# ZeningLin/ViBERTgrid-PyTorch

Hardware: AMD Instinct MI355X
Metric: training docs/sec, 512x512 img + seq_len 512, bert-base+resnet34; 1/2/4/8 GPU (higher is better)
Workload: dtype f32

## Files before the change

include/vbg.h:

```cpp
#ifndef VBG_H
#define VBG_H

#ifdef __cplusplus
extern "C" {
#endif

#define VBG_VERSION 100

int vbg_version(void);

enum {
    VBG_OP_DENSE_K = 0,
    VBG_OP_DENSE_R = 1,
    VBG_OP_CONV_K = 2,
    VBG_OP_CONV_R = 3,
    VBG_OP_WT_R = 4
};
enum { VBG_EPI_NONE = 0, VBG_EPI_RELU = 1, VBG_EPI_GELU_DUAL = 2 ,
       VBG_EPI_MUL_GELU_GRAD = 3  };

typedef struct vbg_conv_geo {
    int Hs, Ws, Cs;
    int Hr, Wr;
    int kh, kw, stride, pad;
// ... 150 lines not shown
int vbg_embed_ln_bwd(const float* dout, const float* xhat, const float* rstd, const int* ids, const int* pos_ids,
                     int ntok, int hidden, const float* gamma, float drop_p, unsigned long long seed,
                     unsigned long long stream_id, float* dword, float* dpos, float* dtype0, float* dgamma,
                     float* dbeta, void* stream);
int vbg_dropout_add_ln_fwd(const float* x, const float* res, int rows, int hidden, const float* gamma,
                           const float* beta, float eps, float drop_p, unsigned long long seed,
                           unsigned long long stream_id, float* y, float* xhat, float* rstd, void* stream);
int vbg_dropout_add_ln_fwd_planes(const float* x, const float* res, int rows, int hidden, const float* gamma,
                                  const float* beta, float eps, float drop_p, unsigned long long seed,
                                  unsigned long long stream_id, float* y, float* xhat, float* rstd, unsigned short* y_planes, int ldp,
                                  long long plane, unsigned short* y_pair, int ldq, long long qplane, void* stream);
int vbg_ln_bwd_ws_rows(int rows);
int vbg_dropout_add_ln_bwd(const float* dy, const float* xhat, const float* rstd, int rows, int hidden,
                           const float* gamma, float drop_p, unsigned long long seed, unsigned long long stream_id,
                           float* dx, float* dres, float* dgamma, float* dbeta, float* slots_ws, unsigned* dx_amax, void* stream);
int vbg_dropout_add_ln_bwd_planes(const float* dy, const float* xhat, const float* rstd, int rows, int hidden,
                                  const float* gamma, float drop_p, unsigned long long seed, unsigned long long stream_id,
                                  unsigned short* dx_planes, int ldp, long long plane, float* dres, float* dgamma, float* dbeta,
                                  float* dbias_accum, float* slots3_ws, void* stream);
int vbg_dropout_add_ln_bwd_pair(const float* dy, const float* xhat, const float* rstd, int rows, int hidden,
                                const float* gamma, float drop_p, unsigned long long seed, unsigned long long stream_id,
                                unsigned short* dx_pair, int ldp, long long plane, float* dres, float* dgamma, float* dbeta,
                                float* dbias_accum, float* slots3_ws, const unsigned* dy_amax, unsigned* dx_amax, unsigned* dx_bound,
                                void* stream);
int vbg_softmax_fwd(float* s, const long long* off, const int* len, const int* ldp, int ngroups, int heads,
                    int maxlen, float scale, float drop_p, unsigned long long seed, unsigned long long stream_id,
                    void* stream);
int vbg_softmax_bwd(const float* p, float* dp, const long long* off, const int* len, const int* ldp, int ngroups,
                    int heads, int maxlen, float scale, float drop_p, void* stream);
int vbg_row_softmax(const float* x, int rows, int cols, float* y, void* stream);
int vbg_gelu_bwd(const float* h, float* dg_inout, long long n, void* stream);
int vbg_relu_bwd(const float* y, float* dy_inout, long long n, void* stream);

typedef struct vbg_planes_ref { unsigned short* buf; long long plane, ld; } vbg_planes_ref;
typedef struct vbg_bert_layer_fwd_desc {
    int ntok, hidden, inter, heads;
    float eps, drop_p; unsigned long long seed, stream_id0;
    int form_qkv, form_attn, form_ao, form_ffn;
    int tile_qkv, tile_ao, tile_ffn1, tile_ffn2;
    int ntasks, max_len; const int* tasks; const int* seq_len; const int* seq_row0; const int* pad_off; long long ntok_pad;
    const unsigned* mask_q; const unsigned* mask_k; const long long* mask_off; float attn_scale, keep_scale;
    const float* x; vbg_planes_ref xa;
    vbg_planes_ref wqkv, wo, wi, wo2;
    const float* bqkv; const float* bo; const float* bi; const float* bo2; const float* g1; const float* b1; const float* g2; const float* b2;
    vbg_planes_ref pqkv;
    float* ctx; float* lse; float* kbar; vbg_planes_ref pctx, pctxq;
    float* ao; float* x1; float* xhat1; float* rstd1; vbg_planes_ref px1, px1q;
    float* h; vbg_planes_ref pg, pgq;
    float* fo; float* y; float* xhat2; float* rstd2; vbg_planes_ref py, pyq;
} vbg_bert_layer_fwd_desc;
int vbg_bert_layer_fwd(const vbg_bert_layer_fwd_desc* desc, void* stream);

int vbg_seg_reduce_fwd(const float* tok, const int* tok_row, const int* run_start, const int* run_len, int nseg,
                       int hidden, int mode, float* out, void* stream);
int vbg_seg_reduce_bwd(const float* dout, const int* tok_row, const int* run_start, const int* run_len, int nseg,
                       int hidden, int mode, float* dtok_accum, void* stream);

int vbg_owner_map(const int* boxes, const int* box_off, int B, int gh, int gw, int stride, int* owner, void* stream);
int vbg_grid_scatter_fwd(const float* emb, const int* owner, int B, int gh, int gw, int C, int layout, float* grid,
                         void* stream);
int vbg_grid_scatter_bwd(const float* dgrid, const int* owner, const int* boxes, const int* box_doc, int nbox, int gh,
                         int gw, int stride, int C, float* demb_accum, void* stream);
int vbg_label_raster(const int* owner, const int* seg_class, long long ncell, int* pos_neg, int* cls, void* stream);

int vbg_bn_slots(void);
int vbg_bn_stats(const float* x, long long M, int C, double* slots_accum, void* stream);
int vbg_bn_finalize(double* stats, int nslots, int clear_slots, double count, const double* count_dev, int C, float eps, float momentum,
                    float* mean, float* invstd, float* running_mean, float* running_var, void* stream);
int vbg_bn_apply(const float* x, const float* res, long long M, int C, const float* mean, const float* invstd,
                 const float* gamma, const float* beta, int relu, float* y, unsigned* y_amax, void* stream);
int vbg_bn_bwd_reduce(const float* dy, const float* y, const float* x, long long M, int C, const float* mean,
                      const float* invstd, int relu, double* slots_accum, void* stream);
int vbg_bn_bwd_apply(const float* dy, const float* y, const float* x, long long M, int C, const float* mean,
                     const float* invstd, const float* gamma, const double* sums, double count, const double* count_dev,
                     int relu, float* dx,
                     float* dres, float* dgamma_accum, float* dbeta_accum, unsigned* dx_amax, void* stream);
int vbg_bn_apply_fold(const float* x, const float* res, long long M, int C, double* slots, int nslots, double count,
                      const double* count_dev, float eps, float momentum, float* mean, float* invstd, float* running_mean,
                      float* running_var, const float* gamma, const float* beta, int relu, float* y, unsigned* y_amax, void* stream);
int vbg_bn_fold_count(double* slots, int nslots, int clear_slots, int C, double* folded, double count, void* stream);
int vbg_bn_bwd_apply_fold(const float* dy, const float* y, const float* x, long long M, int C, const float* mean,
                          const float* invstd, const float* gamma, double* slots, int nslots, double count, int relu, float* dx,
                          float* dres, float* dgamma_accum, float* dbeta_accum, unsigned* dx_amax, void* stream);
int vbg_bn_param_grad(double* slots, int nslots, int clear_slots, int C, double* folded, float* dgamma_accum, float* dbeta_accum,
                      void* stream);
int vbg_maxpool3x3s2_fwd(const float* x, int B, int H, int W, int C, float* y, int* argmax, void* stream);
int vbg_maxpool3x3s2_bwd(const float* dy, const int* argmax, int B, int Ho, int Wo, int C, int H, int W,
                         float* dx, void* stream);
int vbg_avgpool2_fwd(const float* x, int B, int H, int W, int C, float* y, void* stream);
int vbg_avgpool2_bwd(const float* dy, int B, int H, int W, int C, float* dx, void* stream);
int vbg_upsample2_add(const float* lo, const float* skip, int B, int H, int W, int C, float* y, void* stream);
int vbg_sumpool(const float* hi, int B, int H, int W, int C, int f, float* lo, int accumulate, void* stream);
int vbg_nchw_to_nhwc(const float* x, int B, int C, int HW, float* y, void* stream);
int vbg_nhwc_to_nchw(const float* x, int B, int C, int HW, float* y, void* stream);
int vbg_upsample_nhwc_to_nchw(const float* x, int B, int h, int w, int C, int f, float* y, void* stream);
int vbg_add_inplace(float* a, const float* b, long long n, void* stream);

int vbg_roi_align_fwd(const float* feat, int B, int H, int W, int C, const int* boxes, const int* box_doc, int nroi,
                      int out, float scale, float* y , void* stream);
int vbg_roi_align_bwd(const float* dy, int B, int H, int W, int C, const int* boxes, const int* box_doc, int nroi,
                      int out, float scale, float* dfeat_accum, void* stream);
int vbg_roi_align_hw_fwd(const float* feat, int B, int H, int W, int C, const int* boxes, const int* box_doc, int nroi,
                         int out_h, int out_w, float scale, float* y, void* stream);
int vbg_roi_align_hw_bwd(const float* dy, int B, int H, int W, int C, const int* boxes, const int* box_doc, int nroi,
                         int out_h, int out_w, float scale, float* dfeat_accum, void* stream);

int vbg_ce_fwd(const float* logits, long long ld, int ncls, const int* elem, const int* labels, long long n,
               const float* weight, int up_shift, int H, int W, float* loss, void* stream);
int vbg_ce_bwd(const float* logits, long long ld, int ncls, const int* elem, const int* labels, long long n,
               const float* weight, const float* gscale_dev, float gmul, int up_shift, int H, int W,
               float* dlogits_accum, void* stream);
long long vbg_compact_ws_bytes(long long n);
int vbg_compact(const int* labels, long long n, int value, int eq, int* out_idx, int* out_count_dev, void* ws,
                long long ws_bytes, void* stream);
long long vbg_sort_ws_bytes(long long n);
int vbg_sort_desc(const float* keys, long long n, float* keys_out, int* idx_out, void* ws, long long ws_bytes,
                  void* stream);
int vbg_gather_f32(const float* src, const int* idx, long long n, float* out, void* stream);
int vbg_gather_i32(const int* src, const int* idx, long long n, int* out, void* stream);
int vbg_sum_f32(const float* x, long long n, float* out_accum, void* stream);

int vbg_gather_rows(const float* src, const int* idx, long long n, int C, float* dst, void* stream);
int vbg_scatter_rows_add(const float* src, const int* idx, long long n, int C, float* dst_accum, void* stream);
int vbg_crf_nll_fwd(const float* emissions, const int* tags, const int* doc_off, int ndoc, const float* trans, int ntag,
                    int start_tag, int stop_tag, float* alpha, float* logz, float* nll, void* stream);
int vbg_crf_nll_bwd(const float* emissions, const int* tags, const int* doc_off, int ndoc, const float* trans, int ntag,
                    int start_tag, int stop_tag, const float* alpha, const float* logz, const float* gout, float* demissions,
                    float* dtrans_accum, void* stream);
int vbg_crf_viterbi(const float* emissions, const int* doc_off, int ndoc, const float* trans, int ntag, int start_tag,
                    int stop_tag, int* backptr, int* path, float* score, void* stream);

int vbg_sgd_step(float* p, const float* g, float* mom, long long n, float lr, float momentum, float wd,
                 int first_step, float grad_scale, void* stream);
int vbg_adamw_step(float* p, const float* g, float* m, float* v, long long n, float lr, float b1, float b2,
                   float eps, float wd, int step, float grad_scale, void* stream);
int vbg_sumsq(const float* g, long long n, float* out_accum, void* stream);
int vbg_scale_inplace(float* x, long long n, float s, void* stream);

long long vbg_colsum_det_ws_elems(long long M, int N);
int vbg_colsum_det(const float* x, long long ld, long long M, int N, float* out, int accumulate, double* ws, void* stream);
int vbg_sum_det_ws_elems(void);
int vbg_sum_det(const float* x, long long n, int squares, float* out_accum, float* ws, void* stream);
long long vbg_sort_i32_ws_bytes(long long n);
int vbg_sort_i32(const int* keys, long long n, int* keys_out, int* idx_out, void* ws, long long ws_bytes, void* stream);
int vbg_segment_rows_add(const float* src, long long lds, const int* perm, const int* sorted_keys, long long n, int C,
                         float* dst_accum, long long ldd, void* stream);
int vbg_ce_bwd_rows(const float* logits, long long ld, int ncls, const int* elem, const int* labels, long long n,
                    const float* weight, const float* gscale_dev, float gmul, int up_shift, int H, int W, float* grow, int* keys,
                    void* stream);
int vbg_roi_align_bwd_det(const float* dy, int B, int H, int W, int C, const int* boxes, const int* box_doc, int nroi, int out,
                          float scale, float* dfeat_accum, void* stream);
int vbg_roi_align_hw_bwd_det(const float* dy, int B, int H, int W, int C, const int* boxes, const int* box_doc, int nroi, int out_h,
                             int out_w, float scale, float* dfeat_accum, void* stream);
int vbg_bn_det_ws_rows(long long M, int C);
int vbg_bn_stats_det(const float* x, long long M, int C, double* ws, double* zero_slots, void* stream);
int vbg_bn_bwd_reduce_det(const float* dy, const float* y, const float* x, long long M, int C, const float* mean,
                          const float* invstd, int relu, double* ws, double* zero_slots, void* stream);
int vbg_embed_ln_bwd_det_blocks(int ntok);
int vbg_embed_ln_bwd_det(const float* dout, const float* xhat, const float* rstd, int ntok, int hidden, const float* gamma,
                         float drop_p, unsigned long long seed, unsigned long long sid, float* dz_rows, float* part, void* stream);
int vbg_crf_nll_bwd_det(const float* emissions, const int* tags, const int* doc_off, int ndoc, const float* trans, int ntag,
                        int start_tag, int stop_tag, const float* alpha, const float* logz, const float* gout, float* demissions,
                        float* dtrans_part, void* stream);

#ifdef __cplusplus
}
#endif
#endif
```

vibertgrid-pytorch_amd/csrc/convaux.hip:

```cpp
#include "vbg_common.h"
#include "../../include/vbg.h"

namespace vbg {

static inline int ew_grid(long long n, int block) {
    long long g = (n + block - 1) / block;
    if (g > 256 * 8) g = 256 * 8;
    if (g < 1) g = 1;
    return (int)g;
}

constexpr int BN_SLOTS = 32;
template <bool BWD, bool STORE = false>
__global__ __launch_bounds__(256) void bn_reduce_kernel(const float* __restrict__ a, const float* __restrict__ y,
                                                        const float* __restrict__ x, long long M, int C,
                                                        const float* __restrict__ mean, const float* __restrict__ invstd,
                                                        int relu, int rows_per_block, double* out) {
    __shared__ double sh[2][256][4];
    const int C4 = C >> 2;
    const int QB = min(C4, 64);
    const int RL = 256 / QB;
    const int q = threadIdx.x % QB, rl = threadIdx.x / QB;
    const int cq = blockIdx.x * 64 + q;
    const long long r0 = (long long)blockIdx.y * rows_per_block;
    const long long r1 = min(M, r0 + rows_per_block);
    float4 s = make_float4(0.f, 0.f, 0.f, 0.f), t = make_float4(0.f, 0.f, 0.f, 0.f);
    if (cq < C4 && rl < RL) {
        float4 mu = make_float4(0.f, 0.f, 0.f, 0.f), is = mu;
        if (BWD) { mu = reinterpret_cast<const float4*>(mean)[cq]; is = reinterpret_cast<const float4*>(invstd)[cq]; }
#pragma unroll 4
        for (long long r = r0 + rl; r < r1; r += RL) {
            const long long o = r * C4 + cq;
            float4 v = reinterpret_cast<const float4*>(a)[o];
            if (!BWD) {
                s.x += v.x; s.y += v.y; s.z += v.z; s.w += v.w;
                t.x += v.x * v.x; t.y += v.y * v.y; t.z += v.z * v.z; t.w += v.w * v.w;
            } else {
                if (relu) {
                    const float4 yv = reinterpret_cast<const float4*>(y)[o];
                    v.x = yv.x > 0.f ? v.x : 0.f; v.y = yv.y > 0.f ? v.y : 0.f;
                    v.z = yv.z > 0.f ? v.z : 0.f; v.w = yv.w > 0.f ? v.w : 0.f;
                }
                const float4 xv = reinterpret_cast<const float4*>(x)[o];
                s.x += v.x; s.y += v.y; s.z += v.z; s.w += v.w;
                t.x += v.x * ((xv.x - mu.x) * is.x); t.y += v.y * ((xv.y - mu.y) * is.y);
                t.z += v.z * ((xv.z - mu.z) * is.z); t.w += v.w * ((xv.w - mu.w) * is.w);
            }
        }
    }
    sh[0][threadIdx.x][0] = s.x; sh[0][threadIdx.x][1] = s.y; sh[0][threadIdx.x][2] = s.z; sh[0][threadIdx.x][3] = s.w;
    sh[1][threadIdx.x][0] = t.x; sh[1][threadIdx.x][1] = t.y; sh[1][threadIdx.x][2] = t.z; sh[1][threadIdx.x][3] = t.w;
    __syncthreads();
    if (rl == 0 && cq < C4) {
        double a0[4] = {0, 0, 0, 0}, a1[4] = {0, 0, 0, 0};
        for (int l = 0; l < RL; ++l)
#pragma unroll
            for (int j = 0; j < 4; ++j) { a0[j] += sh[0][l * QB + q][j]; a1[j] += sh[1][l * QB + q][j]; }
        double* o = out + (size_t)(STORE ? blockIdx.y : blockIdx.y % BN_SLOTS) * 2 * C;
#pragma unroll
        for (int j = 0; j < 4; ++j) {
            if (STORE) {
                o[cq * 4 + j] = a0[j];
                o[C + cq * 4 + j] = a1[j];
            } else {
                unsafeAtomicAdd(o + cq * 4 + j, a0[j]);
                unsafeAtomicAdd(o + C + cq * 4 + j, a1[j]);
            }
        }
    }
}

static inline int bn_rows_per_block(long long M, int C) {
    const int C4 = C / 4, QB = C4 < 64 ? C4 : 64, RL = 256 / QB, CG = cdiv(C4, 64);
    long long r = cdiv(M * CG, 512);
    if (r < 2 * RL) r = 2 * RL;
    r = cdiv(r, RL) * RL;
    return (int)r;
}

__device__ __forceinline__ double fold_slots(double* __restrict__ slots, int nslots, int C, int idx, bool clear) {
    double v[4] = {0.0, 0.0, 0.0, 0.0};
    int s = 0;
#pragma unroll 2
    for (; s + 3 < nslots; s += 4) {
#pragma unroll
        for (int j = 0; j < 4; ++j) v[j] += slots[(size_t)(s + j) * 2 * C + idx];
    }
    for (; s < nslots; ++s) v[0] += slots[(size_t)s * 2 * C + idx];
    if (clear)
        for (s = 0; s < nslots; ++s) slots[(size_t)s * 2 * C + idx] = 0.0;
    return (v[0] + v[1]) + (v[2] + v[3]);
}

__global__ void bn_finalize_kernel(double* __restrict__ stats, int nslots, int clear, double count, const double* __restrict__ count_dev, int C,
                                   float eps, float momentum, float* mean, float* invstd, float* running_mean,
                                   float* running_var) {
    const int c = blockIdx.x * blockDim.x + threadIdx.x;
    if (c >= C) return;
    if (count_dev) count = count_dev[0];
    const double m = fold_slots(stats, nslots, C, c, clear) / count;
    double var = fold_slots(stats, nslots, C, C + c, clear) / count - m * m;
    if (var < 0.0) var = 0.0;
    mean[c] = (float)m;
    invstd[c] = (float)(1.0 / sqrt(var + (double)eps));
    if (running_mean) {
        const double unbiased = count > 1.0 ? var * count / (count - 1.0) : var;
        running_mean[c] = (1.f - momentum) * running_mean[c] + momentum * (float)m;
        running_var[c] = (1.f - momentum) * running_var[c] + momentum * (float)unbiased;
    }
}

__device__ __forceinline__ void amax_publish(float mx, unsigned* amax) {
    __shared__ float amax_sh[16];
#pragma unroll
    for (int o = 32; o > 0; o >>= 1) mx = fmaxf(mx, __shfl_xor(mx, o, 64));
    if ((threadIdx.x & 63) == 0) amax_sh[threadIdx.x >> 6] = mx;
    __syncthreads();
    if (threadIdx.x == 0) {
        for (int w = 1; w < (int)(blockDim.x >> 6); ++w) mx = fmaxf(mx, amax_sh[w]);
        const unsigned bits = __float_as_uint(mx);
        unsigned* word = amax + (blockIdx.x & (VBG_AMAX_WORDS - 1)) * VBG_AMAX_STRIDE;
        if (bits > __hip_atomic_load(word, __ATOMIC_RELAXED, __HIP_MEMORY_SCOPE_AGENT)) atomicMax(word, bits);
    }
}

__global__ void bn_apply_kernel(const float* __restrict__ x, const float* __restrict__ res, long long M, int C4,
                                const float* __restrict__ mean, const float* __restrict__ invstd,
                                const float* __restrict__ gamma, const float* __restrict__ beta, int relu,
                                float* __restrict__ y, unsigned* amax) {
    const long long total = M * C4;
    const long long stride = (long long)gridDim.x * blockDim.x;
    float mx = 0.f;
    for (long long i = (long long)blockIdx.x * blockDim.x + threadIdx.x; i < total; i += stride) {
        const int c4 = (int)(i % C4);
        const float4 xv = reinterpret_cast<const float4*>(x)[i];
        const float4 mu = reinterpret_cast<const float4*>(mean)[c4];
        const float4 is = reinterpret_cast<const float4*>(invstd)[c4];
        const float4 ga = reinterpret_cast<const float4*>(gamma)[c4];
        const float4 be = reinterpret_cast<const float4*>(beta)[c4];
        float4 o;
        o.x = (xv.x - mu.x) * is.x * ga.x + be.x; o.y = (xv.y - mu.y) * is.y * ga.y + be.y;
        o.z = (xv.z - mu.z) * is.z * ga.z + be.z; o.w = (xv.w - mu.w) * is.w * ga.w + be.w;
        if (res) {
            const float4 rv = reinterpret_cast<const float4*>(res)[i];
            o.x += rv.x; o.y += rv.y; o.z += rv.z; o.w += rv.w;
        }
        if (relu) { o.x = fmaxf(o.x, 0.f); o.y = fmaxf(o.y, 0.f); o.z = fmaxf(o.z, 0.f); o.w = fmaxf(o.w, 0.f); }
        reinterpret_cast<float4*>(y)[i] = o;
        mx = fmaxf(fmaxf(mx, fmaxf(fabsf(o.x), fabsf(o.y))), fmaxf(fabsf(o.z), fabsf(o.w)));
    }
    if (amax) amax_publish(mx, amax);
}

__global__ void bn_bwd_apply_kernel(const float* __restrict__ dy, const float* __restrict__ y, const float* __restrict__ x,
                                    long long M, int C4, int C, const float* __restrict__ mean, const float* __restrict__ invstd,
                                    const float* __restrict__ gamma, const double* __restrict__ sums, double count,
                                    const double* __restrict__ count_dev, int relu, float* __restrict__ dx,
                                    float* __restrict__ dres, unsigned* amax) {
    if (count_dev) count = count_dev[0];
    float mx = 0.f;
    const float icnt = (float)(1.0 / count);
    const long long total = M * C4;
    const long long stride = (long long)gridDim.x * blockDim.x;
    for (long long i = (long long)blockIdx.x * blockDim.x + threadIdx.x; i < total; i += stride) {
        const int c4 = (int)(i % C4), c = c4 * 4;
        float4 g = reinterpret_cast<const float4*>(dy)[i];
        if (relu) {
            const float4 yv = reinterpret_cast<const float4*>(y)[i];
            g.x = yv.x > 0.f ? g.x : 0.f; g.y = yv.y > 0.f ? g.y : 0.f; g.z = yv.z > 0.f ? g.z : 0.f; g.w = yv.w > 0.f ? g.w : 0.f;
        }
        const float4 xv = reinterpret_cast<const float4*>(x)[i];
        const float4 mu = reinterpret_cast<const float4*>(mean)[c4], is = reinterpret_cast<const float4*>(invstd)[c4];
        const float4 ga = reinterpret_cast<const float4*>(gamma)[c4];
        float4 o;
        o.x = ga.x * is.x * (g.x - (float)sums[c + 0] * icnt - (xv.x - mu.x) * is.x * ((float)sums[C + c + 0] * icnt));
        o.y = ga.y * is.y * (g.y - (float)sums[c + 1] * icnt - (xv.y - mu.y) * is.y * ((float)sums[C + c + 1] * icnt));
        o.z = ga.z * is.z * (g.z - (float)sums[c + 2] * icnt - (xv.z - mu.z) * is.z * ((float)sums[C + c + 2] * icnt));
        o.w = ga.w * is.w * (g.w - (float)sums[c + 3] * icnt - (xv.w - mu.w) * is.w * ((float)sums[C + c + 3] * icnt));
        reinterpret_cast<float4*>(dx)[i] = o;
        if (dres) reinterpret_cast<float4*>(dres)[i] = g;
        mx = fmaxf(fmaxf(mx, fmaxf(fabsf(o.x), fabsf(o.y))), fmaxf(fabsf(o.z), fabsf(o.w)));
    }
    if (amax) amax_publish(mx, amax);
}

__device__ __forceinline__ void amax_publish_at(float mx, unsigned* amax, unsigned block_id) {
    __shared__ float amax_sh2[16];
#pragma unroll
    for (int o = 32; o > 0; o >>= 1) mx = fmaxf(mx, __shfl_xor(mx, o, 64));
    if ((threadIdx.x & 63) == 0) amax_sh2[threadIdx.x >> 6] = mx;
    __syncthreads();
    if (threadIdx.x == 0) {
        for (int w = 1; w < (int)(blockDim.x >> 6); ++w) mx = fmaxf(mx, amax_sh2[w]);
        const unsigned bits = __float_as_uint(mx);
        unsigned* word = amax + (block_id & (VBG_AMAX_WORDS - 1)) * VBG_AMAX_STRIDE;
        if (bits > __hip_atomic_load(word, __ATOMIC_RELAXED, __HIP_MEMORY_SCOPE_AGENT)) atomicMax(word, bits);
    }
}

__global__ __launch_bounds__(256) void bn_apply_fold_kernel(const float* __restrict__ x, const float* __restrict__ res, long long M, int C,
                                                            double* __restrict__ slots, int nslots, double count,
                                                            const double* __restrict__ count_dev, float eps, float momentum,
                                                            float* __restrict__ mean_out, float* __restrict__ invstd_out,
                                                            float* __restrict__ running_mean, float* __restrict__ running_var,
                                                            const float* __restrict__ gamma, const float* __restrict__ beta, int relu,
                                                            int rows_per_block, float* __restrict__ y, unsigned* amax) {
    __shared__ double fold[128];
    __shared__ __attribute__((aligned(16))) float cst[4][64];
    const int tid = threadIdx.x, c0 = blockIdx.y * 64;
    if (count_dev) count = count_dev[0];
    if (tid < 128) fold[tid] = fold_slots(slots, nslots, C, (tid >> 6) * C + c0 + (tid & 63), false);
    __syncthreads();
    if (tid < 64) {
        const int c = c0 + tid;
        const double m = fold[tid] / count;
        double var = fold[64 + tid] / count - m * m;
        if (var < 0.0) var = 0.0;
        const float mf = (float)m, isf = (float)(1.0 / sqrt(var + (double)eps));
        cst[0][tid] = mf; cst[1][tid] = isf; cst[2][tid] = gamma[c]; cst[3][tid] = beta[c];
        if (blockIdx.x == 0) {
            mean_out[c] = mf;
            invstd_out[c] = isf;
            if (running_mean) {
                const double unbiased = count > 1.0 ? var * count / (count - 1.0) : var;
                running_mean[c] = (1.f - momentum) * running_mean[c] + momentum * mf;
                running_var[c] = (1.f - momentum) * running_var[c] + momentum * (float)unbiased;
            }
        }
    }
    __syncthreads();
    const int q = tid & 15, rl = tid >> 4, C4 = C >> 2, cq = blockIdx.y * 16 + q;
    const float4 mu = reinterpret_cast<const float4*>(cst[0])[q], is = reinterpret_cast<const float4*>(cst[1])[q];
    const float4 ga = reinterpret_cast<const float4*>(cst[2])[q], be = reinterpret_cast<const float4*>(cst[3])[q];
    const long long r0 = (long long)blockIdx.x * rows_per_block, r1 = min(M, r0 + rows_per_block);
    float mx = 0.f;
#pragma unroll 4
    for (long long r = r0 + rl; r < r1; r += 16) {
        const long long i = r * C4 + cq;
        const float4 xv = reinterpret_cast<const float4*>(x)[i];
        float4 o;
        o.x = (xv.x - mu.x) * is.x * ga.x + be.x; o.y = (xv.y - mu.y) * is.y * ga.y + be.y;
        o.z = (xv.z - mu.z) * is.z * ga.z + be.z; o.w = (xv.w - mu.w) * is.w * ga.w + be.w;
        if (res) {
            const float4 rv = reinterpret_cast<const float4*>(res)[i];
            o.x += rv.x; o.y += rv.y; o.z += rv.z; o.w += rv.w;
        }
        if (relu) { o.x = fmaxf(o.x, 0.f); o.y = fmaxf(o.y, 0.f); o.z = fmaxf(o.z, 0.f); o.w = fmaxf(o.w, 0.f); }
        reinterpret_cast<float4*>(y)[i] = o;
        mx = fmaxf(fmaxf(mx, fmaxf(fabsf(o.x), fabsf(o.y))), fmaxf(fabsf(o.z), fabsf(o.w)));
    }
    if (amax) amax_publish_at(mx, amax, blockIdx.x + blockIdx.y * gridDim.x);
}

__global__ __launch_bounds__(256) void bn_bwd_apply_fold_kernel(const float* __restrict__ dy, const float* __restrict__ y,
                                                                const float* __restrict__ x, long long M, int C,
                                                                const float* __restrict__ mean, const float* __restrict__ invstd,
                                                                const float* __restrict__ gamma, double* __restrict__ slots, int nslots,
                                                                double count, int relu, int rows_per_block, float* __restrict__ dx,
                                                                float* __restrict__ dres, float* dgamma, float* dbeta, unsigned* amax) {
    __shared__ double fold[128];
    __shared__ __attribute__((aligned(16))) float cst[5][64];
    const int tid = threadIdx.x, c0 = blockIdx.y * 64;
    if (tid < 128) fold[tid] = fold_slots(slots, nslots, C, (tid >> 6) * C + c0 + (tid & 63), false);
    __syncthreads();
    const float icnt = (float)(1.0 / count);
    if (tid < 64) {
        const int c = c0 + tid;
        const double sg = fold[tid], sgx = fold[64 + tid];
        cst[0][tid] = mean[c]; cst[1][tid] = invstd[c]; cst[2][tid] = gamma[c];
        cst[3][tid] = (float)sg * icnt; cst[4][tid] = (float)sgx * icnt;
        if (blockIdx.x == 0) {
            if (dbeta) dbeta[c] += (float)sg;
            if (dgamma) dgamma[c] += (float)sgx;
        }
    }
    __syncthreads();
    const int q = tid & 15, rl = tid >> 4, C4 = C >> 2, cq = blockIdx.y * 16 + q;
    const float4 mu = reinterpret_cast<const float4*>(cst[0])[q], is = reinterpret_cast<const float4*>(cst[1])[q];
    const float4 ga = reinterpret_cast<const float4*>(cst[2])[q], s0 = reinterpret_cast<const float4*>(cst[3])[q];
    const float4 s1 = reinterpret_cast<const float4*>(cst[4])[q];
    const long long r0 = (long long)blockIdx.x * rows_per_block, r1 = min(M, r0 + rows_per_block);
    float mx = 0.f;
#pragma unroll 4
    for (long long r = r0 + rl; r < r1; r += 16) {
        const long long i = r * C4 + cq;
        float4 g = reinterpret_cast<const float4*>(dy)[i];
        if (relu) {
            const float4 yv = reinterpret_cast<const float4*>(y)[i];
            g.x = yv.x > 0.f ? g.x : 0.f; g.y = yv.y > 0.f ? g.y : 0.f; g.z = yv.z > 0.f ? g.z : 0.f; g.w = yv.w > 0.f ? g.w : 0.f;
        }
        const float4 xv = reinterpret_cast<const float4*>(x)[i];
        float4 o;
        o.x = ga.x * is.x * (g.x - s0.x - (xv.x - mu.x) * is.x * s1.x);
        o.y = ga.y * is.y * (g.y - s0.y - (xv.y - mu.y) * is.y * s1.y);
        o.z = ga.z * is.z * (g.z - s0.z - (xv.z - mu.z) * is.z * s1.z);
        o.w = ga.w * is.w * (g.w - s0.w - (xv.w - mu.w) * is.w * s1.w);
        reinterpret_cast<float4*>(dx)[i] = o;
        if (dres) reinterpret_cast<float4*>(dres)[i] = g;
        mx = fmaxf(fmaxf(mx, fmaxf(fabsf(o.x), fabsf(o.y))), fmaxf(fabsf(o.z), fabsf(o.w)));
    }
    if (amax) amax_publish_at(mx, amax, blockIdx.x + blockIdx.y * gridDim.x);
}

__global__ __launch_bounds__(256) void amax_kernel(const float* __restrict__ x, long long n, unsigned* amax) {
    const long long n4 = n / 4, stride = (long long)gridDim.x * blockDim.x;
    float mx = 0.f;
    for (long long i = (long long)blockIdx.x * blockDim.x + threadIdx.x; i < n4; i += stride) {
        const float4 v = reinterpret_cast<const float4*>(x)[i];
        mx = fmaxf(fmaxf(mx, fmaxf(fabsf(v.x), fabsf(v.y))), fmaxf(fabsf(v.z), fabsf(v.w)));
    }
    if (blockIdx.x == 0 && threadIdx.x < (int)(n - n4 * 4)) mx = fmaxf(mx, fabsf(x[n4 * 4 + threadIdx.x]));
    amax_publish(mx, amax);
}

__global__ void bn_param_grad_kernel(double* __restrict__ slots, int nslots, int clear, int C, double* __restrict__ folded, float* dgamma,
                                     float* dbeta, double tail = -1.0) {
    const int c = blockIdx.x * blockDim.x + threadIdx.x;
    if (c == 0 && folded && tail >= 0.0) folded[2 * C] = tail;
    if (c >= C) return;
    const double sg = fold_slots(slots, nslots, C, c, clear), sgx = fold_slots(slots, nslots, C, C + c, clear);
    if (folded) { folded[c] = sg; folded[C + c] = sgx; }
    if (dbeta) dbeta[c] += (float)sg;
    if (dgamma) dgamma[c] += (float)sgx;
}

__global__ void maxpool_fwd_kernel(const float* __restrict__ x, int B, int H, int W, int C, int Ho, int Wo,
                                   float* __restrict__ y, int* __restrict__ argmax) {
    const long long total = (long long)B * Ho * Wo * C;
    const long long stride = (long long)gridDim.x * blockDim.x;
    for (long long i = (long long)blockIdx.x * blockDim.x + threadIdx.x; i < total; i += stride) {
        const int c = (int)(i % C);
        long long t = i / C;
        const int ox = (int)(t % Wo); t /= Wo;
        const int oy = (int)(t % Ho);
        const int b = (int)(t / Ho);
        float best = -INFINITY;
        int bi = -1;
        for (int dy = 0; dy < 3; ++dy) {
            const int iy = oy * 2 - 1 + dy;
            if (iy < 0 || iy >= H) continue;
            for (int dx = 0; dx < 3; ++dx) {
                const int ix = ox * 2 - 1 + dx;
                if (ix < 0 || ix >= W) continue;
                const float v = x[(((long long)b * H + iy) * W + ix) * C + c];
                if (v > best || bi < 0) { best = v; bi = iy * W + ix; }
            }
        }
        y[i] = best;
        argmax[i] = bi;
    }
}

__global__ void maxpool_bwd_kernel(const float* __restrict__ dy, const int* __restrict__ argmax, int B, int Ho, int Wo, int C4, int H,
                                   int W, float* __restrict__ dx) {
    const long long total = (long long)B * H * W * C4;
    const long long stride = (long long)gridDim.x * blockDim.x;
    for (long long i = (long long)blockIdx.x * blockDim.x + threadIdx.x; i < total; i += stride) {
        const int c4 = (int)(i % C4);
        long long t = i / C4;
        const int x = (int)(t % W); t /= W;
        const int y = (int)(t % H);
        const int b = (int)(t / H);
        const int me = y * W + x;
        float4 g = make_float4(0.f, 0.f, 0.f, 0.f);
        for (int oy = y >> 1; oy <= ((y + 1) >> 1); ++oy) {
            if (oy >= Ho) continue;
            for (int ox = x >> 1; ox <= ((x + 1) >> 1); ++ox) {
                if (ox >= Wo) continue;
                const long long o = (((long long)b * Ho + oy) * Wo + ox) * C4 + c4;
                const int4 am = reinterpret_cast<const int4*>(argmax)[o];
                const float4 d = reinterpret_cast<const float4*>(dy)[o];
                g.x += am.x == me ? d.x : 0.f; g.y += am.y == me ? d.y : 0.f;
// ... 102 lines not shown
    const long long total = (long long)B * C * H * W;
    const long long stride = (long long)gridDim.x * blockDim.x;
    for (long long i = (long long)blockIdx.x * blockDim.x + threadIdx.x; i < total; i += stride) {
        const int X = (int)(i % W);
        long long t = i / W;
        const int Y = (int)(t % H); t /= H;
        const int c = (int)(t % C);
        const int b = (int)(t / C);
        y[i] = x[(((long long)b * h + Y / f) * w + X / f) * C + c];
    }
}

__global__ void normalize_resize_kernel(const float* __restrict__ img, int h, int w, int oh, int ow, float m0, float m1, float m2,
                                        float s0, float s1, float s2, float* __restrict__ out, int W) {
    const int i = blockIdx.x * blockDim.x + threadIdx.x;
    if (i >= oh * ow) return;
    const int oy = i / ow, ox = i - oy * ow;
    const float mean[3] = {m0, m1, m2}, sd[3] = {s0, s1, s2};
    float v[3];
    if (oh == h && ow == w) {
#pragma unroll
        for (int c = 0; c < 3; ++c) v[c] = (img[((long long)c * h + oy) * w + ox] - mean[c]) / sd[c];
    } else {
        const float sy = (float)h / (float)oh, sx = (float)w / (float)ow;
        float fy = ((float)oy + 0.5f) * sy - 0.5f; if (fy < 0.f) fy = 0.f;
        float fx = ((float)ox + 0.5f) * sx - 0.5f; if (fx < 0.f) fx = 0.f;
        const int y0 = (int)fy, x0 = (int)fx;
        const int y1 = y0 + ((y0 < h - 1) ? 1 : 0), x1 = x0 + ((x0 < w - 1) ? 1 : 0);
        const float ly = fy - (float)y0, lx = fx - (float)x0, hy = 1.f - ly, hx = 1.f - lx;
#pragma unroll
        for (int c = 0; c < 3; ++c) {
            const float* p = img + (long long)c * h * w;
            const float a = (p[(long long)y0 * w + x0] - mean[c]) / sd[c], b = (p[(long long)y0 * w + x1] - mean[c]) / sd[c];
            const float d = (p[(long long)y1 * w + x0] - mean[c]) / sd[c], e = (p[(long long)y1 * w + x1] - mean[c]) / sd[c];
            v[c] = hy * (hx * a + lx * b) + ly * (hx * d + lx * e);
        }
    }
    float* o = out + ((long long)oy * W + ox) * 3;
    o[0] = v[0]; o[1] = v[1]; o[2] = v[2];
}

__global__ void rescale_boxes_kernel(const long long* __restrict__ in, int n, float rh, float rw, int* __restrict__ out) {
    const int i = blockIdx.x * blockDim.x + threadIdx.x;
    if (i >= n) return;
    const float r = ((i & 1) == 0) ? rh : rw;
    out[i] = (int)__fmul_rn((float)in[i], r);
}

__global__ void im2col_kernel(const float* __restrict__ x, int B, int H, int W, int C, int kh, int kw, int stride, int pad,
                              int Ho, int Wo, int Kpad, float* __restrict__ out) {
    const int KQ = Kpad >> 2, K = kh * kw * C;
    const long long total = (long long)B * Ho * Wo * KQ;
    const long long gstride = (long long)gridDim.x * blockDim.x;
    for (long long i = (long long)blockIdx.x * blockDim.x + threadIdx.x; i < total; i += gstride) {
        const long long pix = i / KQ;
        const int k0 = (int)(i - pix * KQ) * 4;
        const int p = (int)pix;
        const int ox = p % Wo, t = p / Wo, oy = t % Ho, b = t / Ho;
        const float* img = x + (long long)b * H * W * C;
        float v[4];
#pragma unroll
        for (int j = 0; j < 4; ++j) {
            const int k = k0 + j;
            v[j] = 0.f;
            if (k < K) {
                const int tap = k / C, c = k - tap * C;
                const int dy = tap / kw, dx = tap - dy * kw;
                const int iy = oy * stride - pad + dy, ix = ox * stride - pad + dx;
                if (iy >= 0 && iy < H && ix >= 0 && ix < W) v[j] = img[(iy * W + ix) * C + c];
            }
        }
        reinterpret_cast<float4*>(out)[i] = make_float4(v[0], v[1], v[2], v[3]);
    }
}

}

using namespace vbg;
#define S_ ((hipStream_t)stream)
#define ALIGNED16(p) (((uintptr_t)(p)) % 16 == 0)

extern "C" int vbg_bn_stats(const float* x, long long M, int C, double* stats_accum, void* stream) {
    VBG_CHECK_ARG(x && stats_accum && M >= 0 && C > 0 && C % 4 == 0 && ALIGNED16(x));
    VBG_CHECK_ARG(C / 4 <= 64 ? (256 % (C / 4) == 0) : (C / 4) % 64 == 0);
    if (M == 0) return VBG_OK;
    const int rpb = bn_rows_per_block(M, C);
    VBG_LAUNCH((bn_reduce_kernel<false>), dim3(cdiv(C / 4, 64), cdiv(M, rpb)), dim3(256), 0, S_, x, nullptr, nullptr, M, C, nullptr,
               nullptr, 0, rpb, stats_accum);
    VBG_LAUNCH_RET();
}

extern "C" int vbg_bn_slots(void) { return BN_SLOTS; }

extern "C" int vbg_bn_finalize(double* stats, int nslots, int clear_slots, double count, const double* count_dev, int C, float eps, float momentum,
                               float* mean, float* invstd, float* running_mean, float* running_var, void* stream) {
    VBG_CHECK_ARG(stats && nslots >= 1 && mean && invstd && C > 0 && (count > 0 || count_dev) &&
                  ((running_mean == nullptr) == (running_var == nullptr)));
    VBG_LAUNCH(bn_finalize_kernel, dim3(cdiv(C, 256)), dim3(256), 0, S_, stats, nslots, clear_slots, count, count_dev, C, eps, momentum, mean,
                       invstd, running_mean, running_var);
    VBG_LAUNCH_RET();
}

extern "C" int vbg_bn_apply(const float* x, const float* res, long long M, int C, const float* mean, const float* invstd,
                            const float* gamma, const float* beta, int relu, float* y, unsigned* y_amax, void* stream) {
    VBG_CHECK_ARG(x && mean && invstd && gamma && beta && y && M >= 0 && C > 0 && C % 4 == 0);
    VBG_CHECK_ARG(ALIGNED16(x) && ALIGNED16(y) && ALIGNED16(mean) && ALIGNED16(invstd) && ALIGNED16(gamma) && ALIGNED16(beta) &&
                  (!res || ALIGNED16(res)));
    if (M == 0) return VBG_OK;
    VBG_LAUNCH(bn_apply_kernel, dim3(ew_grid(M * (C / 4), 256)), dim3(256), 0, S_, x, res, M, C / 4, mean, invstd, gamma,
                       beta, relu, y, y_amax);
    VBG_LAUNCH_RET();
}

extern "C" int vbg_bn_bwd_reduce(const float* dy, const float* y, const float* x, long long M, int C, const float* mean,
                                 const float* invstd, int relu, double* sums_accum, void* stream) {
    VBG_CHECK_ARG(dy && x && mean && invstd && sums_accum && M >= 0 && C > 0 && (!relu || y) && C % 4 == 0);
    VBG_CHECK_ARG(ALIGNED16(dy) && ALIGNED16(x) && ALIGNED16(mean) && ALIGNED16(invstd) && (!relu || ALIGNED16(y)));
    VBG_CHECK_ARG(C / 4 <= 64 ? (256 % (C / 4) == 0) : (C / 4) % 64 == 0);
    if (M == 0) return VBG_OK;
    const int rpb = bn_rows_per_block(M, C);
    VBG_LAUNCH((bn_reduce_kernel<true>), dim3(cdiv(C / 4, 64), cdiv(M, rpb)), dim3(256), 0, S_, dy, y, x, M, C, mean, invstd, relu,
               rpb, sums_accum);
    VBG_LAUNCH_RET();
}

extern "C" int vbg_bn_bwd_apply(const float* dy, const float* y, const float* x, long long M, int C, const float* mean,
                                const float* invstd, const float* gamma, const double* sums, double count,
                                const double* count_dev, int relu, float* dx, float* dres, float* dgamma_accum,
                                float* dbeta_accum, unsigned* dx_amax, void* stream) {
    VBG_CHECK_ARG(dy && x && mean && invstd && gamma && sums && dx && M >= 0 && C > 0 && (count > 0 || count_dev) && (!relu || y));
    VBG_CHECK_ARG(C % 4 == 0 && ALIGNED16(dy) && ALIGNED16(x) && ALIGNED16(dx) && ALIGNED16(mean) && ALIGNED16(invstd) &&
                  ALIGNED16(gamma) && (!relu || ALIGNED16(y)) && (!dres || ALIGNED16(dres)));
    if (M > 0) VBG_LAUNCH(bn_bwd_apply_kernel, dim3(ew_grid(M * (C / 4), 256)), dim3(256), 0, S_, dy, y, x, M, C / 4, C, mean, invstd,
                          gamma, sums, count, count_dev, relu, dx, dres, dx_amax);
    if (dgamma_accum && dbeta_accum)
        VBG_LAUNCH(bn_param_grad_kernel, dim3(cdiv(C, 256)), dim3(256), 0, S_, const_cast<double*>(sums), 1, 0, C, (double*)nullptr, dgamma_accum, dbeta_accum, -1.0);
    VBG_LAUNCH_RET();
}

static inline int bn_fold_rows(long long M, int C) {
    long long r = cdiv(M * (C / 64), 1536);
    if (r < 64) r = 64;
    return (int)(cdiv(r, 16) * 16);
}

extern "C" int vbg_bn_apply_fold(const float* x, const float* res, long long M, int C, double* slots, int nslots, double count,
                                 const double* count_dev, float eps, float momentum, float* mean, float* invstd, float* running_mean,
                                 float* running_var, const float* gamma, const float* beta, int relu, float* y, unsigned* y_amax, void* stream) {
    VBG_CHECK_ARG(x && y && slots && mean && invstd && gamma && beta && M > 0 && C > 0 && C % 64 == 0 && nslots >= 1 && (count > 0 || count_dev));
    VBG_CHECK_ARG((running_mean == nullptr) == (running_var == nullptr) && ALIGNED16(x) && ALIGNED16(y) && (!res || ALIGNED16(res)));
    const int rpb = bn_fold_rows(M, C);
    VBG_LAUNCH(bn_apply_fold_kernel, dim3(cdiv(M, rpb), C / 64), dim3(256), 0, S_, x, res, M, C, slots, nslots, count, count_dev, eps, momentum, mean, invstd,
               running_mean, running_var, gamma, beta, relu, rpb, y, y_amax);
    VBG_LAUNCH_RET();
}

extern "C" int vbg_bn_bwd_apply_fold(const float* dy, const float* y, const float* x, long long M, int C, const float* mean,
                                     const float* invstd, const float* gamma, double* slots, int nslots, double count, int relu, float* dx,
                                     float* dres, float* dgamma_accum, float* dbeta_accum, unsigned* dx_amax, void* stream) {
    VBG_CHECK_ARG(dy && x && mean && invstd && gamma && slots && dx && M > 0 && C > 0 && C % 64 == 0 && nslots >= 1 && count > 0 && (!relu || y));
    VBG_CHECK_ARG(((dgamma_accum == nullptr) == (dbeta_accum == nullptr)) && ALIGNED16(dy) && ALIGNED16(x) && ALIGNED16(dx) &&
                  (!relu || ALIGNED16(y)) && (!dres || ALIGNED16(dres)));
    const int rpb = bn_fold_rows(M, C);
    VBG_LAUNCH(bn_bwd_apply_fold_kernel, dim3(cdiv(M, rpb), C / 64), dim3(256), 0, S_, dy, y, x, M, C, mean, invstd, gamma, slots, nslots, count,
               relu, rpb, dx, dres, dgamma_accum, dbeta_accum, dx_amax);
    VBG_LAUNCH_RET();
}

extern "C" int vbg_amax(const float* x, long long n, unsigned* amax, void* stream) {
    VBG_CHECK_ARG(n >= 0 && amax);
    if (n == 0) return VBG_OK;
    VBG_CHECK_ARG(x && ALIGNED16(x));
    VBG_LAUNCH(amax_kernel, dim3(ew_grid((n + 3) / 4, 256 * 8)), dim3(256), 0, S_, x, n, amax);
    VBG_LAUNCH_RET();
}

extern "C" int vbg_bn_param_grad(double* slots, int nslots, int clear_slots, int C, double* folded, float* dgamma_accum,
                                 float* dbeta_accum, void* stream) {
    VBG_CHECK_ARG(slots && nslots >= 1 && C > 0 && ((dgamma_accum == nullptr) == (dbeta_accum == nullptr)) && (folded || dgamma_accum));
    VBG_LAUNCH(bn_param_grad_kernel, dim3(cdiv(C, 256)), dim3(256), 0, S_, slots, nslots, clear_slots, C, folded, dgamma_accum, dbeta_accum, -1.0);
    VBG_LAUNCH_RET();
}

extern "C" int vbg_bn_fold_count(double* slots, int nslots, int clear_slots, int C, double* folded, double count, void* stream) {
    VBG_CHECK_ARG(slots && folded && nslots >= 1 && C > 0 && count >= 0);
    VBG_LAUNCH(bn_param_grad_kernel, dim3(cdiv(C, 256)), dim3(256), 0, S_, slots, nslots, clear_slots, C, folded, (float*)nullptr, (float*)nullptr, count);
    VBG_LAUNCH_RET();
}

extern "C" int vbg_maxpool3x3s2_fwd(const float* x, int B, int H, int W, int C, float* y, int* argmax, void* stream) {
    VBG_CHECK_ARG(x && y && argmax && B >= 0 && H > 0 && W > 0 && C > 0);
    const int Ho = (H + 2 - 3) / 2 + 1, Wo = (W + 2 - 3) / 2 + 1;
    const long long total = (long long)B * Ho * Wo * C;
    if (total == 0) return VBG_OK;
    VBG_LAUNCH(maxpool_fwd_kernel, dim3(ew_grid(total, 256)), dim3(256), 0, S_, x, B, H, W, C, Ho, Wo, y, argmax);
    VBG_LAUNCH_RET();
}

extern "C" int vbg_maxpool3x3s2_bwd(const float* dy, const int* argmax, int B, int Ho, int Wo, int C, int H, int W,
                                    float* dx_zeroed, void* stream) {
    VBG_CHECK_ARG(dy && argmax && dx_zeroed && B >= 0 && Ho > 0 && Wo > 0 && C > 0 && C % 4 == 0);
    VBG_CHECK_ARG(ALIGNED16(dy) && ALIGNED16(argmax) && ALIGNED16(dx_zeroed) && Ho == (H + 2 - 3) / 2 + 1 && Wo == (W + 2 - 3) / 2 + 1);
    const long long total = (long long)B * Ho * Wo * C;
    if (total == 0) return VBG_OK;
    VBG_LAUNCH(maxpool_bwd_kernel, dim3(ew_grid((long long)B * H * W * (C / 4), 256)), dim3(256), 0, S_, dy, argmax, B, Ho, Wo, C / 4, H, W,
               dx_zeroed);
    VBG_LAUNCH_RET();
}

extern "C" int vbg_upsample2_add(const float* lo, const float* skip, int B, int H, int W, int C, float* y, void* stream) {
    VBG_CHECK_ARG(lo && skip && y && H % 2 == 0 && W % 2 == 0 && C % 4 == 0 && ALIGNED16(lo) && ALIGNED16(skip) && ALIGNED16(y));
    const long long total = (long long)B * H * W * (C / 4);
    if (total == 0) return VBG_OK;
    VBG_LAUNCH(upsample2_add_kernel, dim3(ew_grid(total, 256)), dim3(256), 0, S_, lo, skip, B, H, W, C / 4, y);
    VBG_LAUNCH_RET();
}

extern "C" int vbg_avgpool2_fwd(const float* x, int B, int H, int W, int C, float* y, void* stream) {
    VBG_CHECK_ARG(x && y && B >= 0 && H >= 2 && W >= 2 && C > 0 && C % 4 == 0 && ALIGNED16(x) && ALIGNED16(y));
    const long long total = (long long)B * (H / 2) * (W / 2) * (C / 4);
    if (total == 0) return VBG_OK;
    VBG_LAUNCH((avgpool2_kernel<false>), dim3(ew_grid(total, 256)), dim3(256), 0, S_, x, B, H, W, C / 4, y);
    VBG_LAUNCH_RET();
}

extern "C" int vbg_avgpool2_bwd(const float* dy, int B, int H, int W, int C, float* dx, void* stream) {
    VBG_CHECK_ARG(dy && dx && B >= 0 && H >= 2 && W >= 2 && C > 0 && C % 4 == 0 && ALIGNED16(dy) && ALIGNED16(dx));
    const long long total = (long long)B * H * W * (C / 4);
    if (total == 0) return VBG_OK;
    VBG_LAUNCH((avgpool2_kernel<true>), dim3(ew_grid(total, 256)), dim3(256), 0, S_, dy, B, H, W, C / 4, dx);
    VBG_LAUNCH_RET();
}

extern "C" int vbg_sumpool(const float* hi, int B, int H, int W, int C, int f, float* lo, int accumulate, void* stream) {
    VBG_CHECK_ARG(hi && lo && f >= 1 && H % f == 0 && W % f == 0 && C % 4 == 0 && ALIGNED16(hi) && ALIGNED16(lo));
    const long long total = (long long)B * (H / f) * (W / f) * (C / 4);
    if (total == 0) return VBG_OK;
    VBG_LAUNCH(sumpool_kernel, dim3(ew_grid(total, 256)), dim3(256), 0, S_, hi, B, H, W, C / 4, f, lo, accumulate);
    VBG_LAUNCH_RET();
}

extern "C" int vbg_nchw_to_nhwc(const float* x, int B, int C, int HW, float* y, void* stream) {
    VBG_CHECK_ARG(x && y && B >= 0 && C > 0 && HW > 0);
    if (B == 0) return VBG_OK;
    VBG_LAUNCH(transpose_kernel, dim3(cdiv(HW, 32), cdiv(C, 32), B), dim3(256), 0, S_, x, C, HW, y);
    VBG_LAUNCH_RET();
}

extern "C" int vbg_nhwc_to_nchw(const float* x, int B, int C, int HW, float* y, void* stream) {
    VBG_CHECK_ARG(x && y && B >= 0 && C > 0 && HW > 0);
    if (B == 0) return VBG_OK;
    VBG_LAUNCH(transpose_kernel, dim3(cdiv(C, 32), cdiv(HW, 32), B), dim3(256), 0, S_, x, HW, C, y);
    VBG_LAUNCH_RET();
}

extern "C" int vbg_upsample_nhwc_to_nchw(const float* x, int B, int h, int w, int C, int f, float* y, void* stream) {
    VBG_CHECK_ARG(x && y && f >= 1 && C > 0);
    const long long total = (long long)B * C * h * f * w * f;
    if (total == 0) return VBG_OK;
    VBG_LAUNCH(upsample_nhwc_to_nchw_kernel, dim3(ew_grid(total, 256)), dim3(256), 0, S_, x, B, h, w, C, f, y);
    VBG_LAUNCH_RET();
}

extern "C" int vbg_normalize_resize(const float* img, int h, int w, int oh, int ow, const float* h_mean3, const float* h_std3,
                                    float* batch_nhwc, int b, int H, int W, void* stream) {
    VBG_CHECK_ARG(img && h_mean3 && h_std3 && batch_nhwc && h > 0 && w > 0 && oh > 0 && ow > 0 && oh <= H && ow <= W && b >= 0);
    float* out = batch_nhwc + (long long)b * H * W * 3;
    VBG_LAUNCH(normalize_resize_kernel, dim3(cdiv((long)oh * ow, 256)), dim3(256), 0, S_, img, h, w, oh, ow, h_mean3[0],
                       h_mean3[1], h_mean3[2], h_std3[0], h_std3[1], h_std3[2], out, W);
    VBG_LAUNCH_RET();
}

extern "C" int vbg_rescale_boxes(const long long* in, int S, float ratio_h, float ratio_w, int* out, void* stream) {
    VBG_CHECK_ARG(S >= 0);
    if (S == 0) return VBG_OK;
    VBG_CHECK_ARG(in && out);
    VBG_LAUNCH(rescale_boxes_kernel, dim3(cdiv(S * 4, 256)), dim3(256), 0, S_, in, S * 4, ratio_h, ratio_w, out);
    VBG_LAUNCH_RET();
}

extern "C" int vbg_im2col(const float* x, int B, int H, int W, int C, int kh, int kw, int stride, int pad, int Kpad, float* out,
                          void* stream) {
    VBG_CHECK_ARG(x && out && Kpad >= kh * kw * C && Kpad % 4 == 0 && stride > 0 && ALIGNED16(out));
    const int Ho = (H + 2 * pad - kh) / stride + 1, Wo = (W + 2 * pad - kw) / stride + 1;
    VBG_CHECK_ARG((long long)B * Ho * Wo < (1ll << 31) && (long long)H * W * C < (1ll << 31));
    const long long total = (long long)B * Ho * Wo * (Kpad / 4);
    if (total == 0) return VBG_OK;
    VBG_LAUNCH(im2col_kernel, dim3(ew_grid(total, 256)), dim3(256), 0, S_, x, B, H, W, C, kh, kw, stride, pad, Ho, Wo, Kpad,
                       out);
    VBG_LAUNCH_RET();
}

__global__ void bn_det_fold_kernel(const double* __restrict__ ws, int nblk, int C2, double* __restrict__ slot0) {
    const int i = blockIdx.x * blockDim.x + threadIdx.x;
    if (i >= C2) return;
    double s = 0.0;
    for (int k = 0; k < nblk; ++k) s += ws[(long long)k * C2 + i];
    slot0[i] = s;
}

extern "C" int vbg_bn_det_ws_rows(long long M, int C) {
    if (M <= 0 || C <= 0 || C % 4 != 0) return 0;
    return cdiv(M, bn_rows_per_block(M, C));
}

extern "C" int vbg_bn_stats_det(const float* x, long long M, int C, double* ws, double* zero_slots, void* stream) {
    VBG_CHECK_ARG(x && ws && zero_slots && M >= 0 && C > 0 && C % 4 == 0 && ALIGNED16(x));
    VBG_CHECK_ARG(C / 4 <= 64 ? (256 % (C / 4) == 0) : (C / 4) % 64 == 0);
    if (M == 0) return VBG_OK;
    const int rpb = bn_rows_per_block(M, C), nblk = cdiv(M, rpb);
    VBG_LAUNCH((bn_reduce_kernel<false, true>), dim3(cdiv(C / 4, 64), nblk), dim3(256), 0, S_, x, nullptr, nullptr, M, C, nullptr,
               nullptr, 0, rpb, ws);
    VBG_LAUNCH(bn_det_fold_kernel, dim3(cdiv(2 * C, 256)), dim3(256), 0, S_, ws, nblk, 2 * C, zero_slots);
    VBG_LAUNCH_RET();
}

extern "C" int vbg_bn_bwd_reduce_det(const float* dy, const float* y, const float* x, long long M, int C, const float* mean,
                                     const float* invstd, int relu, double* ws, double* zero_slots, void* stream) {
    VBG_CHECK_ARG(dy && x && mean && invstd && ws && zero_slots && M >= 0 && C > 0 && (!relu || y) && C % 4 == 0);
    VBG_CHECK_ARG(ALIGNED16(dy) && ALIGNED16(x) && ALIGNED16(mean) && ALIGNED16(invstd) && (!relu || ALIGNED16(y)));
    VBG_CHECK_ARG(C / 4 <= 64 ? (256 % (C / 4) == 0) : (C / 4) % 64 == 0);
    if (M == 0) return VBG_OK;
    const int rpb = bn_rows_per_block(M, C), nblk = cdiv(M, rpb);
    VBG_LAUNCH((bn_reduce_kernel<true, true>), dim3(cdiv(C / 4, 64), nblk), dim3(256), 0, S_, dy, y, x, M, C, mean, invstd, relu,
               rpb, ws);
    VBG_LAUNCH(bn_det_fold_kernel, dim3(cdiv(2 * C, 256)), dim3(256), 0, S_, ws, nblk, 2 * C, zero_slots);
    VBG_LAUNCH_RET();
}
```

vibertgrid-pytorch_amd/csrc/gemm_planes.hip:

```cpp
#include "vbg_common.h"
#include <type_traits>
#include <cstdlib>
#include <hip/hip_ext.h>
#include "../../include/vbg.h"

namespace vbg {

typedef unsigned pg_u32x4 __attribute__((ext_vector_type(4)));
typedef __bf16 pg_bf16x8 __attribute__((ext_vector_type(8)));
constexpr unsigned PG_INVALID = 0x80000000u;

__device__ __forceinline__ __amdgpu_buffer_rsrc_t pg_rsrc(const void* base) {
    return __builtin_amdgcn_make_buffer_rsrc(const_cast<void*>(base), 0, (int)0x80000000u, 0x00020000);
}

typedef _Float16 pg_f16x8 __attribute__((ext_vector_type(8)));
__device__ __forceinline__ void pg_split2(float a, float b, unsigned& hi, unsigned& lo) {
    typedef float f32x2_t __attribute__((ext_vector_type(2)));
    typedef _Float16 f16x2_t __attribute__((ext_vector_type(2)));
    const f32x2_t v = {a, b};
    const f16x2_t h = __builtin_convertvector(v, f16x2_t);
    const f16x2_t l = __builtin_convertvector((v - __builtin_convertvector(h, f32x2_t)) * 2048.f, f16x2_t);
    hi = __builtin_bit_cast(unsigned, h);
    lo = __builtin_bit_cast(unsigned, l);
// ... 608 lines not shown
                const float4 hv = *reinterpret_cast<const float4*>(C2 + (long long)gm * ldc + gn);
                v.x *= gelu_erf_grad(hv.x); v.y *= gelu_erf_grad(hv.y); v.z *= gelu_erf_grad(hv.z); v.w *= gelu_erf_grad(hv.w);
            }
            if (C) *reinterpret_cast<float4*>(cp) = v;
            if (epi == VBG_EPI_GELU_DUAL) {
                v = make_float4(gelu_erf(v.x), gelu_erf(v.y), gelu_erf(v.z), gelu_erf(v.w));
                if (C2) *reinterpret_cast<float4*>(C2 + (long long)gm * ldc + gn) = v;
            }
            if (Cp) {
                const float e[4] = {v.x, v.y, v.z, v.w};
                unsigned short h[4], m[4], l[4];
#pragma unroll
                for (int t = 0; t < 4; ++t) pg_split3(e[t], h[t], m[t], l[t]);
                unsigned short* o = Cp + (long long)gm * p.ldp + gn;
                *reinterpret_cast<uint2*>(o) = make_uint2(h[0] | ((unsigned)h[1] << 16), h[2] | ((unsigned)h[3] << 16));
                *reinterpret_cast<uint2*>(o + p.c_plane) = make_uint2(m[0] | ((unsigned)m[1] << 16), m[2] | ((unsigned)m[3] << 16));
                *reinterpret_cast<uint2*>(o + 2 * p.c_plane) = make_uint2(l[0] | ((unsigned)l[1] << 16), l[2] | ((unsigned)l[3] << 16));
            }
        }
        __syncthreads();
    }
}

__device__ __forceinline__ void pg_split3(float x, unsigned short& h, unsigned short& m, unsigned short& l) {
    const unsigned u = __float_as_uint(x);
    const float r1 = x - __uint_as_float(u & 0xffff0000u);
    const unsigned u1 = __float_as_uint(r1);
    const float r2 = r1 - __uint_as_float(u1 & 0xffff0000u);
    h = (unsigned short)(u >> 16); m = (unsigned short)(u1 >> 16); l = (unsigned short)(__float_as_uint(r2) >> 16);
}

__global__ __launch_bounds__(256) void split_planes_kernel(const float* __restrict__ x, long long ldx, int rows, int cols,
                                                            unsigned short* __restrict__ out, int ldp, long long plane, int relu,
                                                            float* colsum) {
    extern __shared__ float sh_cols[];
    const int cpr = ldp / 8;
    const long long n = (long long)rows * cpr;
    const long long stride = (long long)gridDim.x * blockDim.x;
    float cs[8] = {0.f, 0.f, 0.f, 0.f, 0.f, 0.f, 0.f, 0.f};
    const long long i0 = (long long)blockIdx.x * blockDim.x + threadIdx.x;
    for (long long i = i0; i < n; i += stride) {
        const int r = (int)(i / cpr), c = (int)(i % cpr) * 8;
        float e[8];
        if (c + 8 <= cols && ((ldx & 3) == 0) && ((((uintptr_t)x) & 15) == 0)) {
            const float4 a = *reinterpret_cast<const float4*>(x + (long long)r * ldx + c);
            const float4 b = *reinterpret_cast<const float4*>(x + (long long)r * ldx + c + 4);
            e[0] = a.x; e[1] = a.y; e[2] = a.z; e[3] = a.w; e[4] = b.x; e[5] = b.y; e[6] = b.z; e[7] = b.w;
        } else {
#pragma unroll
            for (int t = 0; t < 8; ++t) e[t] = (c + t < cols) ? x[(long long)r * ldx + c + t] : 0.f;
        }
        unsigned short h[8], m[8], l[8];
#pragma unroll
        for (int t = 0; t < 8; ++t) {
            cs[t] += e[t];
            pg_split3(relu ? fmaxf(e[t], 0.f) : e[t], h[t], m[t], l[t]);
        }
        unsigned short* o = out + (long long)r * ldp + c;
        auto pack = [](const unsigned short* s) {
            return make_uint4(s[0] | ((unsigned)s[1] << 16), s[2] | ((unsigned)s[3] << 16), s[4] | ((unsigned)s[5] << 16), s[6] | ((unsigned)s[7] << 16));
        };
        *reinterpret_cast<uint4*>(o) = pack(h);
        *reinterpret_cast<uint4*>(o + plane) = pack(m);
        *reinterpret_cast<uint4*>(o + 2 * plane) = pack(l);
    }
    if (colsum) {
        for (int c = threadIdx.x; c < ldp; c += blockDim.x) sh_cols[c] = 0.f;
        __syncthreads();
        if (i0 < n) {
            const int c = (int)(i0 % cpr) * 8;
#pragma unroll
            for (int t = 0; t < 8; ++t) atomicAdd(&sh_cols[c + t], cs[t]);
        }
        __syncthreads();
        for (int c = threadIdx.x; c < cols; c += blockDim.x) {
            const float v = sh_cols[c];
            if (v != 0.f) unsafeAtomicAdd(colsum + c, v);
        }
    }
}

__global__ __launch_bounds__(256) void split_planes_pair_kernel(const float* __restrict__ x, long long ldx, int rows, int cols,
                                                                 unsigned short* __restrict__ out, int ldp, long long plane,
                                                                 const unsigned* amax, float* colsum) {
    extern __shared__ float sh_cols[];
    const float sc = amax ? vbg_pow2_scale(vbg_amax_read(amax)).x : 1.f;
    float cs[8] = {0.f, 0.f, 0.f, 0.f, 0.f, 0.f, 0.f, 0.f};
    const long long i0 = (long long)blockIdx.x * blockDim.x + threadIdx.x;
    const int cpr = ldp / 8;
    const long long n = (long long)rows * cpr;
    const long long stride = (long long)gridDim.x * blockDim.x;
    const bool vec = ((ldx & 3) == 0) && ((((uintptr_t)x) & 15) == 0);
    for (long long i = (long long)blockIdx.x * blockDim.x + threadIdx.x; i < n; i += stride) {
        const int r = (int)(i / cpr), c = (int)(i % cpr) * 8;
        float e[8];
        if (c + 8 <= cols && vec) {
            const float4 a = *reinterpret_cast<const float4*>(x + (long long)r * ldx + c);
            const float4 b = *reinterpret_cast<const float4*>(x + (long long)r * ldx + c + 4);
            e[0] = a.x; e[1] = a.y; e[2] = a.z; e[3] = a.w; e[4] = b.x; e[5] = b.y; e[6] = b.z; e[7] = b.w;
        } else {
#pragma unroll
            for (int t = 0; t < 8; ++t) e[t] = (c + t < cols) ? x[(long long)r * ldx + c + t] : 0.f;
        }
#pragma unroll
        for (int t = 0; t < 8; ++t) { cs[t] += e[t]; e[t] *= sc; }
        uint4 h, l;
        pg_split2(e[0], e[1], h.x, l.x); pg_split2(e[2], e[3], h.y, l.y); pg_split2(e[4], e[5], h.z, l.z); pg_split2(e[6], e[7], h.w, l.w);
        unsigned short* o = out + (long long)r * ldp + c;
        *reinterpret_cast<uint4*>(o) = h;
        *reinterpret_cast<uint4*>(o + plane) = l;
    }
    if (colsum) {
        for (int c = threadIdx.x; c < ldp; c += blockDim.x) sh_cols[c] = 0.f;
        __syncthreads();
        if (i0 < n) {
            const int c = (int)(i0 % cpr) * 8;
#pragma unroll
            for (int t = 0; t < 8; ++t) atomicAdd(&sh_cols[c + t], cs[t]);
        }
        __syncthreads();
        for (int c = threadIdx.x; c < cols; c += blockDim.x) {
            const float v = sh_cols[c];
            if (v != 0.f) unsafeAtomicAdd(colsum + c, v);
        }
    }
}

__global__ __launch_bounds__(256) void col_l1_max_kernel(const vbg_l1_entry* __restrict__ tab, unsigned* __restrict__ out) {
    const vbg_l1_entry e = tab[blockIdx.y];
    const int c0 = blockIdx.x * 64;
    if (c0 >= e.cols) return;
    const int tx = threadIdx.x & 15, ty = threadIdx.x >> 4;
    const int c = c0 + tx * 4;
    const bool vec = (e.ld & 3) == 0 && ((((uintptr_t)e.w) & 15) == 0) && c + 4 <= e.cols;
    float4 s = make_float4(0.f, 0.f, 0.f, 0.f);
#pragma unroll 4
    for (int r = ty; r < e.rows; r += 16) {
        const float* p = e.w + (long long)r * e.ld + c;
        if (vec) {
            const float4 v = *reinterpret_cast<const float4*>(p);
            s.x += fabsf(v.x); s.y += fabsf(v.y); s.z += fabsf(v.z); s.w += fabsf(v.w);
        } else {
            if (c < e.cols) s.x += fabsf(p[0]);
            if (c + 1 < e.cols) s.y += fabsf(p[1]);
            if (c + 2 < e.cols) s.z += fabsf(p[2]);
            if (c + 3 < e.cols) s.w += fabsf(p[3]);
        }
    }
    __shared__ float4 red[16][16];
    red[ty][tx] = s;
    __syncthreads();
    if (ty == 0) {
        float4 t = red[0][tx];
#pragma unroll
        for (int g = 1; g < 16; ++g) { const float4 v = red[g][tx]; t.x += v.x; t.y += v.y; t.z += v.z; t.w += v.w; }
        float m = fmaxf(fmaxf(t.x, t.y), fmaxf(t.z, t.w));
#pragma unroll
        for (int o = 8; o > 0; o >>= 1) m = fmaxf(m, __shfl_xor(m, o, 64));
        if (tx == 0) atomicMax(out + blockIdx.y, __float_as_uint(m));
    }
}

__global__ __launch_bounds__(256) void split_planes_t_kernel(const float* __restrict__ x, long long ldx, int rows, int cols,
                                                              unsigned short* __restrict__ out, int ldp, long long plane) {
    __shared__ float t[64][65];
    const int r0 = blockIdx.x * 64, c0 = blockIdx.y * 64;
    const int tid = threadIdx.x;
    const bool vec = ((ldx & 3) == 0) && ((((uintptr_t)x) & 15) == 0);
#pragma unroll
    for (int i = 0; i < 4; ++i) {
        const int f = tid + i * 256, r = f / 16, c = (f % 16) * 4;
        float4 v = make_float4(0.f, 0.f, 0.f, 0.f);
        if (r0 + r < rows) {
            const float* src = x + (long long)(r0 + r) * ldx + c0 + c;
            if (vec && c0 + c + 4 <= cols) v = *reinterpret_cast<const float4*>(src);
            else {
                if (c0 + c + 0 < cols) v.x = src[0];
                if (c0 + c + 1 < cols) v.y = src[1];
                if (c0 + c + 2 < cols) v.z = src[2];
                if (c0 + c + 3 < cols) v.w = src[3];
            }
        }
        t[r][c] = v.x; t[r][c + 1] = v.y; t[r][c + 2] = v.z; t[r][c + 3] = v.w;
    }
    __syncthreads();
#pragma unroll
    for (int i = 0; i < 2; ++i) {
        const int f = tid + i * 256, c = f / 8, rg = (f % 8) * 8;
        if (c0 + c >= cols || r0 + rg >= ldp) continue;
        unsigned short h[8], m[8], l[8];
#pragma unroll
        for (int e = 0; e < 8; ++e) pg_split3(t[rg + e][c], h[e], m[e], l[e]);
        unsigned short* o = out + (long long)(c0 + c) * ldp + r0 + rg;
        auto pack = [](const unsigned short* s) {
            return make_uint4(s[0] | ((unsigned)s[1] << 16), s[2] | ((unsigned)s[3] << 16), s[4] | ((unsigned)s[5] << 16), s[6] | ((unsigned)s[7] << 16));
        };
        *reinterpret_cast<uint4*>(o) = pack(h);
        *reinterpret_cast<uint4*>(o + plane) = pack(m);
        *reinterpret_cast<uint4*>(o + 2 * plane) = pack(l);
    }
}

template <bool PAIR>
__global__ __launch_bounds__(256) void split_planes_t_batched_kernel(const float* __restrict__ src, unsigned short* __restrict__ dst,
                                                                      const long long* __restrict__ tbl, int njobs, long long plane) {
    __shared__ float t[64][65];
    int j = 0;
// ... 135 lines not shown
            if (tile == 256128) pg_launch_pair<256, 128, 4, 2, 3, true>(d, s, ev0, ev1);
            else pg_launch_pair<128, 128, 4, 2, 3, true>(d, s, ev0, ev1);
            VBG_LAUNCH_RET();
        }
        if (tile == 256128) pg_launch_pair<256, 128, 4, 2, 3>(d, s, ev0, ev1);
        else if (tile == 128130) pg_launch_pair<128, 128, 2, 4, 3>(d, s, ev0, ev1);
        else if (tile == 128129 || tile == 0) pg_launch_pair<128, 128, 4, 2, 4>(d, s, ev0, ev1);
        else if ((tile == 64064 || tile == 64004) && d.ngroups == 0 && !d.c_amax && !d.cq_ref_in && !d.colsum) {
            if (tile == 64004) pg_launch_pair<64, 64, 2, 2, 4>(d, s, ev0, ev1);
            else pg_launch_pair<64, 64, 2, 2, 3>(d, s, ev0, ev1);
        } else return VBG_EARG;
        VBG_LAUNCH_RET();
    }
    VBG_CHECK_ARG(d.form == 0);
    if (d.trans) {
        if (tile == 256128) pg_launch<256, 128, 4, 2, 2, true>(d, s, (hipEvent_t)e0, (hipEvent_t)e1);
        else if (tile == 128130) pg_launch<128, 128, 2, 4, 3, true>(d, s, (hipEvent_t)e0, (hipEvent_t)e1);
        else pg_launch<128, 128, 4, 2, 3, true>(d, s, (hipEvent_t)e0, (hipEvent_t)e1);
        VBG_LAUNCH_RET();
    }
    if (tile == 0) {
        const long t128 = (long)cdiv(d.M, 128) * cdiv(d.N, 128) * d.splitk;
        tile = (t128 >= 200 && d.N >= 128) ? 128128 : 64064;
    }
    if (tile == 256256) {
        VBG_CHECK_ARG(d.splitk == 1 && !d.accumulate && d.K % 16 == 0);
        const dim3 g(cdiv(d.M, 256), cdiv(d.N, 256));
        (void)hipGetLastError();
        hipEvent_t ev0 = (hipEvent_t)e0, ev1 = (hipEvent_t)e1;
        if (ev0 && ev1) hipExtLaunchKernelGGL(plane_gemm_256_kernel, g, dim3(512), 0, s, ev0, ev1, 0, d);
        else hipLaunchKernelGGL(plane_gemm_256_kernel, g, dim3(512), 0, s, d);
        VBG_LAUNCH_RET();
    }
    if (tile == 256128) pg_launch<256, 128, 4, 2, 2>(d, s, (hipEvent_t)e0, (hipEvent_t)e1);
    else if (tile == 128128) pg_launch<128, 128, 2, 2, 3>(d, s, (hipEvent_t)e0, (hipEvent_t)e1);
    else if (tile == 128129) pg_launch<128, 128, 4, 2, 3>(d, s, (hipEvent_t)e0, (hipEvent_t)e1);
    else if (tile == 128130) pg_launch<128, 128, 2, 4, 3>(d, s, (hipEvent_t)e0, (hipEvent_t)e1);
    else if (tile == 128064) pg_launch<128, 64, 2, 2, 3>(d, s, (hipEvent_t)e0, (hipEvent_t)e1);
    else if (tile == 64064) pg_launch<64, 64, 2, 2, 3>(d, s, (hipEvent_t)e0, (hipEvent_t)e1);
    else return VBG_EARG;
    VBG_LAUNCH_RET();
}

extern "C" int vbg_plane_gemm(const vbg_plane_gemm_desc* desc, void* stream) { return plane_gemm_dispatch(desc, stream, nullptr, nullptr); }

extern "C" int vbg_plane_gemm_timed(const vbg_plane_gemm_desc* desc, void* stream, void* start_event, void* stop_event) {
    VBG_CHECK_ARG(start_event && stop_event);
    return plane_gemm_dispatch(desc, stream, start_event, stop_event);
}

extern "C" int vbg_split_planes(const float* x, long long ldx, int rows, int cols, unsigned short* out, int ldp, long long plane,
                                int relu, float* colsum_accum, void* stream) {
    VBG_CHECK_ARG(rows >= 0 && cols >= 0 && ldp % 32 == 0 && ldp >= cols && plane >= (long long)rows * ldp && plane % 8 == 0);
    if (rows == 0 || cols == 0) return VBG_OK;
    VBG_CHECK_ARG(x && out && ((uintptr_t)out & 15) == 0);
    const long long n = (long long)rows * (ldp / 8);
    long long g = (n + 255) / 256;
    size_t lds = 0;
    if (colsum_accum) {
        VBG_CHECK_ARG(relu == 0 && ldp * 4 <= 64 * 1024);
        const long long cpr = ldp / 8;
        long long a = cpr, b = 256;
        while (b) { const long long t = a % b; a = b; b = t; }
        const long long unit = cpr / a;
        long long k = 288 / unit;
        if (k < 1) k = 1;
        const long long need = (g + unit - 1) / unit;
        if (k > need) k = need;
        g = k * unit;
        lds = (size_t)ldp * 4;
    } else if (g > 256 * 16) {
        g = 256 * 16;
    }
    VBG_LAUNCH(split_planes_kernel, dim3((unsigned)g), dim3(256), lds, (hipStream_t)stream, x, ldx, rows, cols, out, ldp, plane, relu,
               colsum_accum);
    VBG_LAUNCH_RET();
}

extern "C" int vbg_split_planes_pair(const float* x, long long ldx, int rows, int cols, unsigned short* out, int ldp, long long plane,
                                     const unsigned* amax, float* colsum_accum, void* stream) {
    VBG_CHECK_ARG(rows >= 0 && cols >= 0 && ldp % 32 == 0 && ldp >= cols && plane >= (long long)rows * ldp && plane % 8 == 0);
    if (rows == 0 || cols == 0) return VBG_OK;
    VBG_CHECK_ARG(x && out && ((uintptr_t)out & 15) == 0);
    const long long n = (long long)rows * (ldp / 8);
    long long g = (n + 255) / 256;
    size_t lds = 0;
    if (colsum_accum) {
        VBG_CHECK_ARG(ldp * 4 <= 64 * 1024);
        const long long cpr = ldp / 8;
        long long a = cpr, b = 256;
        while (b) { const long long t = a % b; a = b; b = t; }
        const long long unit = cpr / a;
        long long k = 288 / unit;
        if (k < 1) k = 1;
        const long long need = (g + unit - 1) / unit;
        if (k > need) k = need;
        g = k * unit;
        lds = (size_t)ldp * 4;
    } else if (g > 256 * 16) {
        g = 256 * 16;
    }
    VBG_LAUNCH(split_planes_pair_kernel, dim3((unsigned)g), dim3(256), lds, (hipStream_t)stream, x, ldx, rows, cols, out, ldp, plane, amax, colsum_accum);
    VBG_LAUNCH_RET();
}

extern "C" int vbg_col_l1_max(const vbg_l1_entry* table_dev, int n, int max_cols, unsigned* out, void* stream) {
    VBG_CHECK_ARG(n >= 0 && max_cols >= 0);
    if (n == 0 || max_cols == 0) return VBG_OK;
    VBG_CHECK_ARG(table_dev && out);
    VBG_LAUNCH(col_l1_max_kernel, dim3((unsigned)((max_cols + 63) / 64), (unsigned)n), dim3(256), 0, (hipStream_t)stream, table_dev, out);
    VBG_LAUNCH_RET();
}

extern "C" int vbg_split_planes_t(const float* x, long long ldx, int rows, int cols, unsigned short* out, int ldp, long long plane,
                                  void* stream) {
    VBG_CHECK_ARG(rows >= 0 && cols >= 0 && ldp % 32 == 0 && ldp >= rows && plane >= (long long)cols * ldp && plane % 8 == 0);
    if (rows == 0 || cols == 0) return VBG_OK;
    VBG_CHECK_ARG(x && out && ((uintptr_t)out & 15) == 0);
    VBG_LAUNCH(split_planes_t_kernel, dim3(cdiv(ldp, 64), cdiv(cols, 64)), dim3(256), 0, (hipStream_t)stream, x, ldx, rows, cols, out, ldp, plane);
    VBG_LAUNCH_RET();
}

extern "C" int vbg_split_planes_t_batched(const float* src, unsigned short* dst, const long long* tbl_dev, int njobs, int total_tiles,
                                          long long plane, void* stream) {
    VBG_CHECK_ARG(njobs >= 0 && total_tiles >= 0);
    if (njobs == 0 || total_tiles == 0) return VBG_OK;
    VBG_CHECK_ARG(src && dst && tbl_dev && ((uintptr_t)dst & 15) == 0 && plane % 8 == 0);
    VBG_LAUNCH(split_planes_t_batched_kernel<false>, dim3(total_tiles), dim3(256), 0, (hipStream_t)stream, src, dst, tbl_dev, njobs, plane);
    VBG_LAUNCH_RET();
}

extern "C" int vbg_split_planes_pair_t_batched(const float* src, unsigned short* dst, const long long* tbl_dev, int njobs, int total_tiles,
                                               long long plane, void* stream) {
    VBG_CHECK_ARG(njobs >= 0 && total_tiles >= 0);
    if (njobs == 0 || total_tiles == 0) return VBG_OK;
    VBG_CHECK_ARG(src && dst && tbl_dev && ((uintptr_t)dst & 15) == 0 && plane % 8 == 0);
    VBG_LAUNCH(split_planes_t_batched_kernel<true>, dim3(total_tiles), dim3(256), 0, (hipStream_t)stream, src, dst, tbl_dev, njobs, plane);
    VBG_LAUNCH_RET();
}
```

vibertgrid-pytorch_amd/vbg/functions.py:

```python
from types import SimpleNamespace
from typing import NamedTuple

import torch
import torch.distributed as dist

from . import ops
from .lib import ATTN_DKV, ATTN_DQ, EPI_GELU_DUAL, EPI_MUL_GELU_GRAD, EPI_NONE, EPI_RELU, OP_DENSE_K, OP_DENSE_R

f32 = torch.float32


def ohwi(w):
    v = w.permute(0, 2, 3, 1)
    return v if v.is_contiguous() else v.contiguous()


def oihw_grad_like(dw_ohwi):
    return dw_ohwi.permute(0, 3, 1, 2)


def _c(t):
    return t if t.is_contiguous() else t.contiguous()


# ... 231 lines not shown
        Cout, kh, kw, Cin = w4_shape
        K = kh * kw * Cin
        Mpix = col.shape[0]
        sk = ops._pick_splitk(Cout, K, Mpix)
        if sk > 1:
            dw.zero_()
        ops.gemm_raw(Cout, K, Mpix, dy, Cout, OP_DENSE_R, col, col.shape[1], OP_DENSE_R, dw, K, accumulate=sk > 1, splitk=sk)
    else:
        ops.conv2d_wgrad(dy, x, dw, stride, pad, accumulate=False, dy_amax=dy_amax, x_amax=x_amax)
    return oihw_grad_like(dw)


class ConvFn(torch.autograd.Function):

    @staticmethod
    def forward(ctx, x, w, b, stride, pad):
        ctx.x_amax = _amax_tag(x)
        x = _c(x)
        w4 = ohwi(w)
        y, col, _ = _conv_any(x, w4, stride, pad, b, w_owner=w, x_amax=ctx.x_amax)
        ctx.stride, ctx.pad, ctx.has_bias = stride, pad, b is not None
        ctx.side_ok = SIDE_OK[0]
        ctx.w_ref, ctx.b_ref = w, b
        ctx.save_for_backward(x, w4, col)
        return y

    @staticmethod
    def backward(ctx, dy):
        x, w4, col = ctx.saved_tensors
        dy = _c(dy)
        B_, H_, W_, Cin_ = x.shape
        Cout_, kh, kw, _ = w4.shape
        f16_d = ctx.needs_input_grad[0] and ops.conv3_f16_bwd_ok(B_, H_, W_, Cout_, Cin_, kh, kw, ctx.stride, ctx.pad)
        f16_w = col is None and ops.conv3_f16_wgrad_ok(B_, H_, W_, Cin_, Cout_, kh, kw, ctx.stride, ctx.pad)
        dy_amax = ops.amax(dy) if (f16_d or f16_w) else None
        if ctx.side_ok and ctx.needs_input_grad[0] and sinks(ctx.w_ref) and ops.conv_wgrad_stream_enabled(2, dy.numel() // dy.shape[-1]):
            cur, ws = torch.cuda.current_stream(dy.device), ops.side_stream(dy.device, "cwgrad")
            ws.wait_stream(cur)
            with torch.cuda.stream(ws):
                dw = _conv_wgrad_any(dy, x, col, tuple(w4.shape), ctx.stride, ctx.pad, ctx.w_ref, dy_amax=dy_amax, x_amax=ctx.x_amax)
                ops.reserve_for(ws, dy, x, col, dy_amax, ctx.x_amax)
            assert dw is None
        else:
            dw = _conv_wgrad_any(dy, x, col, tuple(w4.shape), ctx.stride, ctx.pad, ctx.w_ref, dy_amax=dy_amax, x_amax=ctx.x_amax)
        dx = ops.conv2d_dgrad(dy, w4, tuple(x.shape), ctx.stride, ctx.pad, dy_amax=dy_amax, w_owner=ctx.w_ref) if ctx.needs_input_grad[0] else None
        db = _bias_grad(ctx.b_ref, dy.view(-1, dy.shape[-1])) if ctx.has_bias else None
        return dx, dw, db, None, None


def _frozen_invstd(running_var, eps):
    tag = (running_var._version, ops.bn_epoch(), running_var.data_ptr(), float(eps))
    hit = running_var.__dict__.get("_vbg_invstd")
    if hit is not None and hit[0] == tag:
        return hit[1]
    with torch.no_grad():
        inv = torch.rsqrt(running_var + eps)
    running_var.__dict__["_vbg_invstd"] = (tag, inv)
    return inv


class ConvBnFn(torch.autograd.Function):

    @staticmethod
    def forward(ctx, x, w, gamma, beta, running_mean, running_var, res, stride, pad, relu, training, momentum, eps, sync):
        ctx.x_amax = _amax_tag(x)
        x = _c(x)
        sync = bool(sync) and SyncCtx.active()
        w4 = ohwi(w)
        fold = training and ops.bn_fold_ok(w.shape[0], sync)
        if ops.bn_epilogue_route(training, ctx.needs_input_grad, sync):
            y_amax = ops.amax_slot(x.device) if ops.conv3_f16_enabled() else None
            r = None if res is None else _c(res)
            y, _, _ = _conv_any(x, w4, stride, pad, w_owner=w, x_amax=ctx.x_amax,
                                bn=ops.BnEpi(running_mean, _frozen_invstd(running_var, eps), gamma, beta, r, relu, y_amax))
            if y_amax is not None:
                y._vbg_amax = (y_amax, y._version)
            return y
        z, col, stats = _conv_any(x, w4, stride, pad, want_stats=training, w_owner=w, x_amax=ctx.x_amax, zero_slots=fold)
        C = z.shape[-1]
        z2 = z.view(-1, C)
        M = z2.shape[0]
        r2 = None if res is None else _c(res).view(-1, C)
        y_amax = ops.amax_slot(x.device) if (ops.conv3_f16_enabled() or (any(ctx.needs_input_grad) and ops.conv3_f16_bwd_enabled())) else None
        if fold:
            if stats is None:
                stats = ops.bn_stats(z2, ops.bn_zero_slots(x.device, C))
            count, count_dev = float(M), None
            y, mean, invstd = ops.bn_apply_fold(z2, r2, stats, count, eps, momentum, running_mean, running_var, gamma, beta, relu, y_amax=y_amax)
            y = y.view(z.shape)
        else:
            if training:
                if stats is None:
                    stats = ops.bn_stats(z2)
                count, count_dev = float(M), None
                if sync:
                    glob = ops.bn_fold_count(stats, C, M)
                    SyncCtx.all_reduce(glob)
                    count_dev = glob[2 * C:]
                    if ops.bn_fold_ok(C):
                        y, mean, invstd = ops.bn_apply_fold(z2, r2, glob, count, eps, momentum, running_mean, running_var, gamma, beta, relu,
                                                            y_amax=y_amax, nslots=1, count_dev=count_dev)
                        y = y.view(z.shape)
                    else:
                        mean, invstd = ops.bn_finalize(glob, C, 1, count, eps, momentum, running_mean, running_var, count_dev)
                else:
                    mean, invstd = ops.bn_finalize(stats, C, ops.bn_slots(), count, eps, momentum, running_mean, running_var)
            else:
                mean, invstd, count, count_dev = running_mean, _frozen_invstd(running_var, eps), float(M), None
            if not (training and sync and ops.bn_fold_ok(C)):
                y = ops.bn_apply(z2, r2, mean, invstd, gamma, beta, relu, y_amax=y_amax).view(z.shape)
        if y_amax is not None:
            y._vbg_amax = (y_amax, y._version)
        ctx.fold = fold
        ctx.side_ok = SIDE_OK[0]
        ctx.cfg = (stride, pad, relu, training, count, res is not None, sync)
        ctx.w_ref, ctx.affine = w, (gamma, beta)
        ctx.save_for_backward(x, w4, col, z, y if relu else None, mean, invstd, gamma, count_dev)
        return y

    @staticmethod
    def backward(ctx, dy):
        x, w4, col, z, y, mean, invstd, gamma, count_dev = ctx.saved_tensors
        stride, pad, relu, training, count, has_res, sync = ctx.cfg
        C = z.shape[-1]
        dy2 = _c(dy).view(-1, C)
        z2 = z.view(-1, C)
        y2 = None if y is None else y.view(-1, C)
        B_, H_, W_, Cin_ = x.shape
        want_amax = (ctx.needs_input_grad[0] and ops.conv3_f16_bwd_ok(B_, H_, W_, C, Cin_, w4.shape[1], w4.shape[2], stride, pad)) or \
            (col is None and ops.conv3_f16_wgrad_ok(B_, H_, W_, Cin_, C, w4.shape[1], w4.shape[2], stride, pad))
        dz_amax = ops.amax_slot(dy2.device) if want_amax else None
        dgamma, dbeta, sunk = _affine_dest(*ctx.affine)
        if ctx.fold and ops.bn_fold_ok(C, sync):
            slots = ops.bn_bwd_reduce(dy2, y2, z2, mean, invstd, relu, ops.bn_zero_slots(dy2.device, C))
            dz2, dres2 = ops.bn_bwd_apply_fold(dy2, y2, z2, mean, invstd, gamma, slots, count, relu, has_res, dgamma, dbeta, dx_amax=dz_amax)
            dgamma, dbeta = _affine_done(*ctx.affine, dgamma, dbeta, sunk)
            return ConvBnFn._finish_backward(ctx, dz2, dres2, dz_amax, dgamma, dbeta)
        slots = ops.bn_bwd_reduce(dy2, y2, z2, mean, invstd, relu)
        sums = ops.bn_param_grad(slots, C, dgamma, dbeta)
        dgamma, dbeta = _affine_done(*ctx.affine, dgamma, dbeta, sunk)
        if not training:
            sums = torch.zeros_like(sums)
        elif sync:
            SyncCtx.all_reduce(sums)
        dz2, dres2 = ops.bn_bwd_apply(dy2, y2, z2, mean, invstd, gamma, sums, count, relu, has_res, None, None, count_dev, dx_amax=dz_amax)
        return ConvBnFn._finish_backward(ctx, dz2, dres2, dz_amax, dgamma, dbeta)

    @staticmethod
    def _finish_backward(ctx, dz2, dres2, dz_amax, dgamma, dbeta):
        x, w4, col, z, y, mean, invstd, gamma, count_dev = ctx.saved_tensors
        stride, pad, relu, training, count, has_res, sync = ctx.cfg
        dz = dz2.view(z.shape)
        dres = dres2.view(z.shape) if has_res else None
        if ctx.side_ok and ctx.needs_input_grad[0] and sinks(ctx.w_ref) and ops.conv_wgrad_stream_enabled(1, dz2.shape[0]):
            cur, ws = torch.cuda.current_stream(dz.device), ops.side_stream(dz.device, "cwgrad")
            ws.wait_stream(cur)
            with torch.cuda.stream(ws):
                dw = _conv_wgrad_any(dz, x, col, tuple(w4.shape), stride, pad, ctx.w_ref, dy_amax=dz_amax, x_amax=ctx.x_amax)
                ops.reserve_for(ws, dz2, x, col, dz_amax, ctx.x_amax)
            assert dw is None
            dx = ops.conv2d_dgrad(dz, w4, tuple(x.shape), stride, pad, dy_amax=dz_amax, w_owner=ctx.w_ref)
            return dx, None, dgamma, dbeta, None, None, dres, None, None, None, None, None, None, None
        dx = ops.conv2d_dgrad(dz, w4, tuple(x.shape), stride, pad, dy_amax=dz_amax, w_owner=ctx.w_ref) if ctx.needs_input_grad[0] else None
        dw = _conv_wgrad_any(dz, x, col, tuple(w4.shape), stride, pad, ctx.w_ref, dy_amax=dz_amax, x_amax=ctx.x_amax)
        return dx, dw, dgamma, dbeta, None, None, dres, None, None, None, None, None, None, None


class MaxPoolFn(torch.autograd.Function):
    @staticmethod
    def forward(ctx, x):
        x = _c(x)
        y, am = ops.maxpool_fwd(x)
        ctx.hw = (x.shape[1], x.shape[2])
        ctx.save_for_backward(am)
        return y

    @staticmethod
    def backward(ctx, dy):
        (am,) = ctx.saved_tensors
        return ops.maxpool_bwd(_c(dy), am, *ctx.hw)


class AvgPool2Fn(torch.autograd.Function):

    @staticmethod
    def forward(ctx, x):
        x = _c(x)
        ctx.hw = (x.shape[1], x.shape[2])
        return ops.avgpool2_fwd(x)

    @staticmethod
    def backward(ctx, dy):
        return ops.avgpool2_bwd(_c(dy), *ctx.hw)


class UpAddFn(torch.autograd.Function):

    @staticmethod
    def forward(ctx, lo, skip):
        return ops.upsample2_add(_c(lo), _c(skip))

    @staticmethod
    def backward(ctx, dy):
        dy = _c(dy)
        return ops.sumpool(dy, 2), dy


class NhwcToNchwFlatFn(torch.autograd.Function):

    @staticmethod
    def forward(ctx, x):
        ctx.shape = x.shape
        return ops.nhwc_to_nchw(_c(x)).view(x.shape[0], -1)

    @staticmethod
    def backward(ctx, dy):
        N, h, w, C = ctx.shape
        return ops.nchw_to_nhwc(_c(dy).view(N, C, h, w))


class RoiAlignFn(torch.autograd.Function):
    @staticmethod
    def forward(ctx, feat, boxes, box_doc, out_size, scale):
        feat = _c(feat)
        ctx.cfg = (tuple(feat.shape), out_size, scale)
        ctx.save_for_backward(boxes, box_doc)
        return ops.roi_align_fwd(feat, boxes, box_doc, out_size, scale)

# ... 602 lines not shown
```

vibertgrid-pytorch_amd/vbg/lib.py:

```python
import ctypes as C
import os

import torch

_HERE = os.path.dirname(os.path.abspath(__file__))
LIB_PATH = os.environ.get("VBG_LIB_PATH") or os.path.join(os.path.dirname(_HERE), "libvbg.so")

c_int, c_ll, c_f, c_d, c_vp, c_ull = C.c_int, C.c_longlong, C.c_float, C.c_double, C.c_void_p, C.c_ulonglong


class ConvGeo(C.Structure):
    _fields_ = [("Hs", c_int), ("Ws", c_int), ("Cs", c_int), ("Hr", c_int), ("Wr", c_int), ("kh", c_int), ("kw", c_int),
                ("stride", c_int), ("pad", c_int), ("dgrad", c_int)]


class BnEpilogue(C.Structure):
    _fields_ = [("mean", c_vp), ("invstd", c_vp), ("gamma", c_vp), ("beta", c_vp), ("res", c_vp), ("relu", c_int), ("amax", c_vp)]


class GemmDesc(C.Structure):
    _fields_ = [("M", c_int), ("N", c_int), ("K", c_int),
                ("A", c_vp), ("lda", c_ll), ("a_kind", c_int), ("a_vec", c_int),
                ("a_nseg", c_int), ("a_seg_ptr", c_vp * 4), ("a_seg_kend", c_int * 4), ("a_seg_ld", c_ll * 4),
                ("a_seg_shift", c_int * 4), ("a_H", c_int), ("a_W", c_int),
# ... 56 lines not shown
                ("mask_q", c_vp), ("mask_k", c_vp), ("mask_off", c_vp), ("attn_scale", c_f), ("keep_scale", c_f),
                ("x", c_vp), ("xa", PlanesRef),
                ("wqkv", PlanesRef), ("wo", PlanesRef), ("wi", PlanesRef), ("wo2", PlanesRef),
                ("bqkv", c_vp), ("bo", c_vp), ("bi", c_vp), ("bo2", c_vp), ("g1", c_vp), ("b1", c_vp), ("g2", c_vp), ("b2", c_vp),
                ("pqkv", PlanesRef),
                ("ctx", c_vp), ("lse", c_vp), ("kbar", c_vp), ("pctx", PlanesRef), ("pctxq", PlanesRef),
                ("ao", c_vp), ("x1", c_vp), ("xhat1", c_vp), ("rstd1", c_vp), ("px1", PlanesRef), ("px1q", PlanesRef),
                ("h", c_vp), ("pg", PlanesRef), ("pgq", PlanesRef),
                ("fo", c_vp), ("y", c_vp), ("xhat2", c_vp), ("rstd2", c_vp), ("py", PlanesRef), ("pyq", PlanesRef)]


ATTN_FWD, ATTN_DQ, ATTN_DKV = 0, 1, 2
OP_DENSE_K, OP_DENSE_R, OP_CONV_K, OP_CONV_R, OP_WT_R = 0, 1, 2, 3, 4
EPI_NONE, EPI_RELU, EPI_GELU_DUAL, EPI_MUL_GELU_GRAD = 0, 1, 2, 3

SIGNATURES = {
    "vbg_version": (c_int, []),
    "vbg_gemm": (c_int, [C.POINTER(GemmDesc), c_vp]),
    "vbg_gemm_timed": (c_int, [C.POINTER(GemmDesc), c_vp, c_vp, c_vp]),
    "vbg_timer_create": (c_int, [c_vp]),
    "vbg_timer_destroy": (c_int, [c_vp]),
    "vbg_timer_elapsed_ms": (c_int, [c_vp, c_vp, c_vp]),
    "vbg_slab_reduce": (c_int, [c_vp, c_int, c_ll, c_int, c_int, c_ll, c_vp, c_int, c_vp, c_ll, c_vp]),
    "vbg_plane_gemm": (c_int, [C.POINTER(PlaneGemmDesc), c_vp]),
    "vbg_plane_gemm_timed": (c_int, [C.POINTER(PlaneGemmDesc), c_vp, c_vp, c_vp]),
    "vbg_split_planes": (c_int, [c_vp, c_ll, c_int, c_int, c_vp, c_int, c_ll, c_int, c_vp, c_vp]),
    "vbg_col_l1_max": (c_int, [c_vp, c_int, c_int, c_vp, c_vp]),
    "vbg_split_planes_pair": (c_int, [c_vp, c_ll, c_int, c_int, c_vp, c_int, c_ll, c_vp, c_vp, c_vp]),
    "vbg_split_planes_t": (c_int, [c_vp, c_ll, c_int, c_int, c_vp, c_int, c_ll, c_vp]),
    "vbg_split_planes_t_batched": (c_int, [c_vp, c_vp, c_vp, c_int, c_int, c_ll, c_vp]),
    "vbg_split_planes_pair_t_batched": (c_int, [c_vp, c_vp, c_vp, c_int, c_int, c_ll, c_vp]),
    "vbg_attn": (c_int, [C.POINTER(AttnDesc), c_vp]),
    "vbg_bert_layer_fwd": (c_int, [C.POINTER(BertLayerFwdDesc), c_vp]),
    "vbg_attn_drop_thr16": (C.c_uint, [c_f]),
    "vbg_attn_mask": (c_int, [c_vp, c_vp, c_int, c_int, c_int, c_f, c_ull, c_ull, c_vp, c_vp, c_vp]),
    "vbg_attn_mask_layers": (c_int, [c_vp, c_vp, c_int, c_int, c_int, c_f, c_ull, c_ull, c_ull, c_int, c_ll, c_vp, c_vp, c_vp]),
    "vbg_colsum": (c_int, [c_vp, c_ll, c_int, c_int, c_vp, c_int, c_vp]),
    "vbg_colsum_f64": (c_int, [c_vp, c_ll, c_int, c_int, c_vp, c_int, c_vp, c_vp]),
    "vbg_conv3x3": (c_int, [c_vp, c_vp, c_vp, c_vp, c_vp, c_int, c_int, c_int, c_int, c_int, c_int, c_int, c_int, c_vp, c_vp, c_vp, c_int, c_vp]),
    "vbg_conv3x3_bn": (c_int, [c_vp, c_vp, c_vp, c_vp, c_int, c_int, c_int, c_int, c_int, c_int, c_vp, c_vp, c_vp, c_int, c_int, c_vp, c_vp]),
    "vbg_conv3x3_split": (c_int, [c_int, c_int, c_int, c_int, c_int]),
    "vbg_conv3x3_pw": (c_int, [c_vp, c_vp, c_vp, c_vp, c_vp, c_int, c_int, c_int, c_int, c_int, c_int, c_int, c_vp, c_vp, c_vp, c_int, c_int, c_vp]),
    "vbg_conv3x3_pw_amp": (c_int, [c_vp, c_vp, c_vp, c_vp, c_vp, c_int, c_int, c_int, c_int, c_int, c_int, c_int, c_vp, c_vp, c_vp, c_int, c_int, c_vp]),
    "vbg_conv3x3_wprep": (c_int, [c_vp, c_vp, c_int, c_vp]),
    "vbg_conv3x3_wprep_bytes": (c_ll, [c_int, c_int, c_int, c_int]),
    "vbg_amax": (c_int, [c_vp, c_ll, c_vp, c_vp]),
    "vbg_conv3x3_wflip": (c_int, [c_vp, c_int, c_int, c_vp, c_vp]),
    "vbg_conv3x3_wgrad_strips": (c_int, [c_int, c_int, c_int, c_int, c_int]),
    "vbg_conv3x3_wgrad": (c_int, [c_vp, c_vp, c_vp, c_vp, c_int, c_int, c_int, c_int, c_int, c_int, c_vp, c_vp, c_vp]),
    "vbg_im2col": (c_int, [c_vp, c_int, c_int, c_int, c_int, c_int, c_int, c_int, c_int, c_int, c_vp, c_vp]),
    "vbg_normalize_resize": (c_int, [c_vp, c_int, c_int, c_int, c_int, C.POINTER(c_f), C.POINTER(c_f), c_vp, c_int, c_int, c_int, c_vp]),
    "vbg_rescale_boxes": (c_int, [c_vp, c_int, c_f, c_f, c_vp, c_vp]),
    "vbg_embed_ln_fwd": (c_int, [c_vp, c_vp, c_int, c_int, c_vp, c_vp, c_vp, c_vp, c_vp, c_f, c_f, c_ull, c_ull, c_vp, c_vp, c_vp, c_vp]),
    "vbg_embed_ln_bwd": (c_int, [c_vp, c_vp, c_vp, c_vp, c_vp, c_int, c_int, c_vp, c_f, c_ull, c_ull, c_vp, c_vp, c_vp, c_vp, c_vp, c_vp]),
    "vbg_dropout_add_ln_fwd": (c_int, [c_vp, c_vp, c_int, c_int, c_vp, c_vp, c_f, c_f, c_ull, c_ull, c_vp, c_vp, c_vp, c_vp]),
    "vbg_dropout_add_ln_fwd_planes": (c_int, [c_vp, c_vp, c_int, c_int, c_vp, c_vp, c_f, c_f, c_ull, c_ull, c_vp, c_vp, c_vp, c_vp, c_int, c_ll, c_vp, c_int, c_ll, c_vp]),
    "vbg_ln_bwd_ws_rows": (c_int, [c_int]),
    "vbg_dropout_add_ln_bwd": (c_int, [c_vp, c_vp, c_vp, c_int, c_int, c_vp, c_f, c_ull, c_ull, c_vp, c_vp, c_vp, c_vp, c_vp, c_vp, c_vp]),
    "vbg_dropout_add_ln_bwd_pair": (c_int, [c_vp, c_vp, c_vp, c_int, c_int, c_vp, c_f, c_ull, c_ull, c_vp, c_int, c_ll, c_vp, c_vp, c_vp, c_vp, c_vp, c_vp, c_vp, c_vp, c_vp]),
    "vbg_dropout_add_ln_bwd_planes": (c_int, [c_vp, c_vp, c_vp, c_int, c_int, c_vp, c_f, c_ull, c_ull, c_vp, c_int, c_ll, c_vp, c_vp, c_vp, c_vp, c_vp, c_vp]),
    "vbg_softmax_fwd": (c_int, [c_vp, c_vp, c_vp, c_vp, c_int, c_int, c_int, c_f, c_f, c_ull, c_ull, c_vp]),
    "vbg_softmax_bwd": (c_int, [c_vp, c_vp, c_vp, c_vp, c_vp, c_int, c_int, c_int, c_f, c_f, c_vp]),
    "vbg_row_softmax": (c_int, [c_vp, c_int, c_int, c_vp, c_vp]),
    "vbg_gelu_bwd": (c_int, [c_vp, c_vp, c_ll, c_vp]),
    "vbg_relu_bwd": (c_int, [c_vp, c_vp, c_ll, c_vp]),
    "vbg_add_inplace": (c_int, [c_vp, c_vp, c_ll, c_vp]),
    "vbg_scale_inplace": (c_int, [c_vp, c_ll, c_f, c_vp]),
    "vbg_seg_reduce_fwd": (c_int, [c_vp, c_vp, c_vp, c_vp, c_int, c_int, c_int, c_vp, c_vp]),
    "vbg_seg_reduce_bwd": (c_int, [c_vp, c_vp, c_vp, c_vp, c_int, c_int, c_int, c_vp, c_vp]),
    "vbg_owner_map": (c_int, [c_vp, c_vp, c_int, c_int, c_int, c_int, c_vp, c_vp]),
    "vbg_grid_scatter_fwd": (c_int, [c_vp, c_vp, c_int, c_int, c_int, c_int, c_int, c_vp, c_vp]),
    "vbg_grid_scatter_bwd": (c_int, [c_vp, c_vp, c_vp, c_vp, c_int, c_int, c_int, c_int, c_int, c_vp, c_vp]),
    "vbg_label_raster": (c_int, [c_vp, c_vp, c_ll, c_vp, c_vp, c_vp]),
    "vbg_bn_stats": (c_int, [c_vp, c_ll, c_int, c_vp, c_vp]),
    "vbg_bn_slots": (c_int, []),
    "vbg_bn_finalize": (c_int, [c_vp, c_int, c_int, c_d, c_vp, c_int, c_f, c_f, c_vp, c_vp, c_vp, c_vp, c_vp]),
    "vbg_bn_apply": (c_int, [c_vp, c_vp, c_ll, c_int, c_vp, c_vp, c_vp, c_vp, c_int, c_vp, c_vp, c_vp]),
    "vbg_bn_bwd_reduce": (c_int, [c_vp, c_vp, c_vp, c_ll, c_int, c_vp, c_vp, c_int, c_vp, c_vp]),
    "vbg_bn_bwd_apply": (c_int, [c_vp, c_vp, c_vp, c_ll, c_int, c_vp, c_vp, c_vp, c_vp, c_d, c_vp, c_int, c_vp, c_vp, c_vp, c_vp, c_vp, c_vp]),
    "vbg_bn_param_grad": (c_int, [c_vp, c_int, c_int, c_int, c_vp, c_vp, c_vp, c_vp]),
    "vbg_bn_apply_fold": (c_int, [c_vp, c_vp, c_ll, c_int, c_vp, c_int, c_d, c_vp, c_f, c_f, c_vp, c_vp, c_vp, c_vp, c_vp, c_vp, c_int, c_vp, c_vp, c_vp]),
    "vbg_bn_fold_count": (c_int, [c_vp, c_int, c_int, c_int, c_vp, c_d, c_vp]),
    "vbg_bn_bwd_apply_fold": (c_int, [c_vp, c_vp, c_vp, c_ll, c_int, c_vp, c_vp, c_vp, c_vp, c_int, c_d, c_int, c_vp, c_vp, c_vp, c_vp, c_vp, c_vp]),
    "vbg_maxpool3x3s2_fwd": (c_int, [c_vp, c_int, c_int, c_int, c_int, c_vp, c_vp, c_vp]),
    "vbg_maxpool3x3s2_bwd": (c_int, [c_vp, c_vp, c_int, c_int, c_int, c_int, c_int, c_int, c_vp, c_vp]),
    "vbg_avgpool2_fwd": (c_int, [c_vp, c_int, c_int, c_int, c_int, c_vp, c_vp]),
    "vbg_avgpool2_bwd": (c_int, [c_vp, c_int, c_int, c_int, c_int, c_vp, c_vp]),
    "vbg_upsample2_add": (c_int, [c_vp, c_vp, c_int, c_int, c_int, c_int, c_vp, c_vp]),
    "vbg_sumpool": (c_int, [c_vp, c_int, c_int, c_int, c_int, c_int, c_vp, c_int, c_vp]),
    "vbg_nchw_to_nhwc": (c_int, [c_vp, c_int, c_int, c_int, c_vp, c_vp]),
    "vbg_nhwc_to_nchw": (c_int, [c_vp, c_int, c_int, c_int, c_vp, c_vp]),
    "vbg_upsample_nhwc_to_nchw": (c_int, [c_vp, c_int, c_int, c_int, c_int, c_int, c_vp, c_vp]),
    "vbg_roi_align_fwd": (c_int, [c_vp, c_int, c_int, c_int, c_int, c_vp, c_vp, c_int, c_int, c_f, c_vp, c_vp]),
    "vbg_roi_align_bwd": (c_int, [c_vp, c_int, c_int, c_int, c_int, c_vp, c_vp, c_int, c_int, c_f, c_vp, c_vp]),
    "vbg_roi_align_hw_fwd": (c_int, [c_vp, c_int, c_int, c_int, c_int, c_vp, c_vp, c_int, c_int, c_int, c_f, c_vp, c_vp]),
    "vbg_roi_align_hw_bwd": (c_int, [c_vp, c_int, c_int, c_int, c_int, c_vp, c_vp, c_int, c_int, c_int, c_f, c_vp, c_vp]),
    "vbg_ce_fwd": (c_int, [c_vp, c_ll, c_int, c_vp, c_vp, c_ll, c_vp, c_int, c_int, c_int, c_vp, c_vp]),
    "vbg_ce_bwd": (c_int, [c_vp, c_ll, c_int, c_vp, c_vp, c_ll, c_vp, c_vp, c_f, c_int, c_int, c_int, c_vp, c_vp]),
    "vbg_compact_ws_bytes": (c_ll, [c_ll]),
    "vbg_compact": (c_int, [c_vp, c_ll, c_int, c_int, c_vp, c_vp, c_vp, c_ll, c_vp]),
    "vbg_sort_ws_bytes": (c_ll, [c_ll]),
    "vbg_sort_desc": (c_int, [c_vp, c_ll, c_vp, c_vp, c_vp, c_ll, c_vp]),
    "vbg_gather_f32": (c_int, [c_vp, c_vp, c_ll, c_vp, c_vp]),
    "vbg_gather_i32": (c_int, [c_vp, c_vp, c_ll, c_vp, c_vp]),
    "vbg_sum_f32": (c_int, [c_vp, c_ll, c_vp, c_vp]),
    "vbg_sumsq": (c_int, [c_vp, c_ll, c_vp, c_vp]),
    "vbg_gather_rows": (c_int, [c_vp, c_vp, c_ll, c_int, c_vp, c_vp]),
    "vbg_scatter_rows_add": (c_int, [c_vp, c_vp, c_ll, c_int, c_vp, c_vp]),
    "vbg_crf_nll_fwd": (c_int, [c_vp, c_vp, c_vp, c_int, c_vp, c_int, c_int, c_int, c_vp, c_vp, c_vp, c_vp]),
    "vbg_crf_nll_bwd": (c_int, [c_vp, c_vp, c_vp, c_int, c_vp, c_int, c_int, c_int, c_vp, c_vp, c_vp, c_vp, c_vp, c_vp]),
    "vbg_crf_viterbi": (c_int, [c_vp, c_vp, c_int, c_vp, c_int, c_int, c_int, c_vp, c_vp, c_vp, c_vp]),
    "vbg_sgd_step": (c_int, [c_vp, c_vp, c_vp, c_ll, c_f, c_f, c_f, c_int, c_f, c_vp]),
    "vbg_adamw_step": (c_int, [c_vp, c_vp, c_vp, c_vp, c_ll, c_f, c_f, c_f, c_f, c_f, c_int, c_f, c_vp]),
    "vbg_colsum_det_ws_elems": (c_ll, [c_ll, c_int]),
    "vbg_colsum_det": (c_int, [c_vp, c_ll, c_ll, c_int, c_vp, c_int, c_vp, c_vp]),
    "vbg_sum_det_ws_elems": (c_int, []),
    "vbg_sum_det": (c_int, [c_vp, c_ll, c_int, c_vp, c_vp, c_vp]),
    "vbg_sort_i32_ws_bytes": (c_ll, [c_ll]),
    "vbg_sort_i32": (c_int, [c_vp, c_ll, c_vp, c_vp, c_vp, c_ll, c_vp]),
    "vbg_segment_rows_add": (c_int, [c_vp, c_ll, c_vp, c_vp, c_ll, c_int, c_vp, c_ll, c_vp]),
    "vbg_ce_bwd_rows": (c_int, [c_vp, c_ll, c_int, c_vp, c_vp, c_ll, c_vp, c_vp, c_f, c_int, c_int, c_int, c_vp, c_vp, c_vp]),
    "vbg_roi_align_bwd_det": (c_int, [c_vp, c_int, c_int, c_int, c_int, c_vp, c_vp, c_int, c_int, c_f, c_vp, c_vp]),
    "vbg_roi_align_hw_bwd_det": (c_int, [c_vp, c_int, c_int, c_int, c_int, c_vp, c_vp, c_int, c_int, c_int, c_f, c_vp, c_vp]),
    "vbg_bn_det_ws_rows": (c_int, [c_ll, c_int]),
    "vbg_bn_stats_det": (c_int, [c_vp, c_ll, c_int, c_vp, c_vp, c_vp]),
    "vbg_bn_bwd_reduce_det": (c_int, [c_vp, c_vp, c_vp, c_ll, c_int, c_vp, c_vp, c_int, c_vp, c_vp, c_vp]),
    "vbg_embed_ln_bwd_det_blocks": (c_int, [c_int]),
    "vbg_embed_ln_bwd_det": (c_int, [c_vp, c_vp, c_vp, c_int, c_int, c_vp, c_f, c_ull, c_ull, c_vp, c_vp, c_vp]),
    "vbg_crf_nll_bwd_det": (c_int, [c_vp, c_vp, c_vp, c_int, c_vp, c_int, c_int, c_int, c_vp, c_vp, c_vp, c_vp, c_vp, c_vp]),
}


class VbgError(RuntimeError):
    pass


def _load():
    if not os.path.exists(LIB_PATH):
        raise ImportError(
            f"{LIB_PATH} not found: the HIP library is the product and there is no fallback. "
            "Build it with `make -C vibertgrid-pytorch_amd/csrc` (hipcc, gfx950).")
    lib = C.CDLL(LIB_PATH)
    for name, (res, args) in SIGNATURES.items():
        fn = getattr(lib, name)
        fn.restype = res
        fn.argtypes = args
    return lib


lib = _load()


def check(rc: int, what: str):
    if rc != 0:
        kind = "argument error" if rc < 0 else f"hipError {rc}"
        raise VbgError(f"{what} failed: {kind}")
```

vibertgrid-pytorch_amd/vbg/ops.py:

```python
import ctypes as C

import os

import torch

from .lib import (ATTN_FWD, EPI_GELU_DUAL, EPI_NONE, EPI_RELU, OP_CONV_K, OP_CONV_R, OP_DENSE_K, OP_DENSE_R, OP_WT_R, ConvGeo,
                  AttnDesc, BertLayerFwdDesc, BnEpilogue, GemmDesc, PlaneGemmDesc, VbgError, check, lib)

f32 = torch.float32
i32 = torch.int32


def raw_stream(device=None) -> int:
    idx = None if device is None else torch.device(device).index
    return torch._C._cuda_getCurrentRawStream(torch._C._cuda_getDevice() if idx is None else idx)


def _stream():
    return C.c_void_p(torch._C._cuda_getCurrentRawStream(torch._C._cuda_getDevice()))


_OVERLAP = [os.environ.get("VBG_OVERLAP", "1") != "0"]
_SIDE = {}

# ... 1500 lines not shown
def scale_(a, s):
    check(lib.vbg_scale_inplace(P(a), a.numel(), float(s), _stream()), "vbg_scale_inplace")
    return a


def seg_reduce_fwd(tok, tok_row, run_start, run_len, mode):
    nseg, hidden = run_start.numel(), tok.shape[1]
    out = torch.empty((nseg, hidden), device=tok.device, dtype=f32)
    check(lib.vbg_seg_reduce_fwd(P(tok), P(tok_row), P(run_start), P(run_len), nseg, hidden, mode, P(out), _stream()), "vbg_seg_reduce_fwd")
    return out


def seg_reduce_bwd(dout, tok_row, run_start, run_len, mode, dtok):
    nseg, hidden = dout.shape
    check(lib.vbg_seg_reduce_bwd(P(dout), P(tok_row), P(run_start), P(run_len), nseg, hidden, mode, P(dtok), _stream()), "vbg_seg_reduce_bwd")


def owner_map(boxes, box_off, B, gh, gw, stride):
    own = torch.empty((B, gh, gw), device=box_off.device, dtype=i32)
    check(lib.vbg_owner_map(P(boxes) if boxes.numel() else None, P(box_off), B, gh, gw, stride, P(own), _stream()), "vbg_owner_map")
    return own


def grid_scatter_fwd(emb, owner, C_, layout=0):
    B, gh, gw = owner.shape
    shape = (B, gh, gw, C_) if layout == 0 else (B, C_, gh, gw)
    grid = torch.empty(shape, device=owner.device, dtype=f32)
    check(lib.vbg_grid_scatter_fwd(P(emb) if emb.numel() else None, P(owner), B, gh, gw, C_, layout, P(grid), _stream()), "vbg_grid_scatter_fwd")
    return grid


def grid_scatter_bwd(dgrid, owner, boxes, box_doc, stride, demb):
    B, gh, gw = owner.shape
    nbox, C_ = demb.shape
    check(lib.vbg_grid_scatter_bwd(P(dgrid), P(owner), P(boxes) if nbox else None, P(box_doc) if nbox else None, nbox, gh, gw, stride,
                                   C_, P(demb), _stream()), "vbg_grid_scatter_bwd")


def label_raster(owner, seg_class):
    pn = torch.empty_like(owner)
    cl = torch.empty_like(owner)
    check(lib.vbg_label_raster(P(owner), P(seg_class) if seg_class.numel() else None, owner.numel(), P(pn), P(cl), _stream()), "vbg_label_raster")
    return pn, cl


_BN_SLOTS = [0]


def bn_slots():
    if not _BN_SLOTS[0]:
        _BN_SLOTS[0] = int(lib.vbg_bn_slots())
    return _BN_SLOTS[0]


_BN_WS = {}


def _bn_workspace(device, C_):
    key = (device, C_, raw_stream(device))
    ws = _BN_WS.get(key)
    if ws is None:
        ws = _BN_WS[key] = torch.zeros((bn_slots() * 2 * C_,), device=device, dtype=torch.float64)
    return ws


_BN_ZPOOL = {}


def bn_fold_ok(C_, sync=False) -> bool:
    return not sync and C_ % 64 == 0


def bn_zero_slots(device, C_):
    key = (device, raw_stream(device))
    n = bn_slots() * 2 * C_
    ent = _BN_ZPOOL.get(key)
    if ent is None or ent[1] + n > ent[0].numel():
        ent = _BN_ZPOOL[key] = [torch.zeros((max(1 << 20, n),), device=device, dtype=torch.float64), 0]
    o = ent[1]
    ent[1] = o + n
    return ent[0][o:o + n]


def bn_fold_count(slots, C_, count):
    out = torch.empty((2 * C_ + 1,), device=slots.device, dtype=torch.float64)
    check(lib.vbg_bn_fold_count(P(slots), bn_slots(), 1, C_, P(out), float(count), _stream()), "vbg_bn_fold_count")
    return out


def bn_apply_fold(x2d, res2d, slots, count, eps, momentum, running_mean, running_var, gamma, beta, relu, y_amax=None, nslots=None, count_dev=None):
    M, C_ = x2d.shape
    out = torch.empty_like(x2d)
    mean = torch.empty((C_,), device=x2d.device, dtype=f32)
    invstd = torch.empty_like(mean)
    check(lib.vbg_bn_apply_fold(P(x2d), P(res2d), M, C_, P(slots), bn_slots() if nslots is None else int(nslots), float(count), P(count_dev), eps, momentum,
                                P(mean), P(invstd), P(running_mean), P(running_var), P(gamma), P(beta), int(relu), P(out), P(y_amax), _stream()),
          "vbg_bn_apply_fold")
    if running_var is not None:
        _BN_EPOCH[0] += 1
    return out, mean, invstd


def bn_bwd_apply_fold(dy, y, x, mean, invstd, gamma, slots, count, relu, want_dres, dgamma, dbeta, dx_amax=None):
    M, C_ = x.shape
    dx = torch.empty_like(x)
    dres = torch.empty_like(x) if want_dres else None
    check(lib.vbg_bn_bwd_apply_fold(P(dy), P(y), P(x), M, C_, P(mean), P(invstd), P(gamma), P(slots), bn_slots(), float(count), int(relu), P(dx),
                                    P(dres), P(dgamma), P(dbeta), P(dx_amax), _stream()), "vbg_bn_bwd_apply_fold")
    return dx, dres


def _bn_det_ws(device, M, C_):
    return torch.empty((max(int(lib.vbg_bn_det_ws_rows(M, C_)), 1) * 2 * C_,), device=device, dtype=torch.float64)


def bn_stats(x2d, stats=None):
    M, C_ = x2d.shape
    if stats is None:
        stats = _bn_workspace(x2d.device, C_)
    if _DET[0]:
        ws = _bn_det_ws(x2d.device, M, C_)
        check(lib.vbg_bn_stats_det(P(x2d), M, C_, P(ws), P(stats), _stream()), "vbg_bn_stats_det")
        _seen("det:bn_reduce")
        return stats
    _seen("fatomic:bn_reduce")
    check(lib.vbg_bn_stats(P(x2d), M, C_, P(stats), _stream()), "vbg_bn_stats")
    return stats


def bn_fold(slots, C_, out=None):
    if out is None:
        out = torch.empty((2 * C_,), device=slots.device, dtype=torch.float64)
    check(lib.vbg_bn_param_grad(P(slots), bn_slots(), 1, C_, P(out), None, None, _stream()), "vbg_bn_param_grad")
    return out


def bn_finalize(stats, C_, nslots, count, eps, momentum, running_mean, running_var, count_dev=None):
    mean = torch.empty((C_,), device=stats.device, dtype=f32)
    invstd = torch.empty_like(mean)
    check(lib.vbg_bn_finalize(P(stats), int(nslots), int(nslots > 1), float(count), P(count_dev), C_, eps, momentum, P(mean), P(invstd),
                              P(running_mean), P(running_var), _stream()), "vbg_bn_finalize")
    if running_var is not None:
        _BN_EPOCH[0] += 1
    return mean, invstd


_BN_EPOCH = [0]


def bn_epoch() -> int:
    return _BN_EPOCH[0]


def bn_apply(x2d, res2d, mean, invstd, gamma, beta, relu, out=None, y_amax=None):
    M, C_ = x2d.shape
    if out is None:
        out = torch.empty_like(x2d)
    _seen("bn:apply")
    check(lib.vbg_bn_apply(P(x2d), P(res2d), M, C_, P(mean), P(invstd), P(gamma), P(beta), int(relu), P(out), P(y_amax), _stream()), "vbg_bn_apply")
    return out


def bn_bwd_reduce(dy, y, x, mean, invstd, relu, sums=None):
    M, C_ = x.shape
    if sums is None:
        sums = _bn_workspace(x.device, C_)
    if _DET[0]:
        ws = _bn_det_ws(x.device, M, C_)
        check(lib.vbg_bn_bwd_reduce_det(P(dy), P(y), P(x), M, C_, P(mean), P(invstd), int(relu), P(ws), P(sums), _stream()),
              "vbg_bn_bwd_reduce_det")
        _seen("det:bn_reduce")
        return sums
    _seen("fatomic:bn_reduce")
    check(lib.vbg_bn_bwd_reduce(P(dy), P(y), P(x), M, C_, P(mean), P(invstd), int(relu), P(sums), _stream()), "vbg_bn_bwd_reduce")
    return sums


def bn_bwd_apply(dy, y, x, mean, invstd, gamma, sums, count, relu, want_dres, dgamma, dbeta, count_dev=None, dx_amax=None):
    M, C_ = x.shape
    dx = torch.empty_like(x)
    dres = torch.empty_like(x) if want_dres else None
    check(lib.vbg_bn_bwd_apply(P(dy), P(y), P(x), M, C_, P(mean), P(invstd), P(gamma), P(sums), float(count), P(count_dev), int(relu), P(dx), P(dres),
                               P(dgamma), P(dbeta), P(dx_amax), _stream()), "vbg_bn_bwd_apply")
    return dx, dres


def bn_param_grad(slots, C_, dgamma, dbeta):
    folded = torch.empty((2 * C_,), device=slots.device, dtype=torch.float64)
    check(lib.vbg_bn_param_grad(P(slots), bn_slots(), 1, C_, P(folded), P(dgamma), P(dbeta), _stream()), "vbg_bn_param_grad")
    return folded


def maxpool_fwd(x):
    B, H, W, C_ = x.shape
    Ho, Wo = conv_out_hw(H, W, 3, 2, 1)
    y = torch.empty((B, Ho, Wo, C_), device=x.device, dtype=f32)
    am = torch.empty((B, Ho, Wo, C_), device=x.device, dtype=i32)
    check(lib.vbg_maxpool3x3s2_fwd(P(x), B, H, W, C_, P(y), P(am), _stream()), "vbg_maxpool_fwd")
    return y, am


def maxpool_bwd(dy, am, H, W):
    B, Ho, Wo, C_ = dy.shape
    dx = torch.empty((B, H, W, C_), device=dy.device, dtype=f32)
    check(lib.vbg_maxpool3x3s2_bwd(P(dy), P(am), B, Ho, Wo, C_, H, W, P(dx), _stream()), "vbg_maxpool_bwd")
    return dx


def avgpool2_fwd(x):
    B, H, W, C_ = x.shape
    y = torch.empty((B, H // 2, W // 2, C_), device=x.device, dtype=f32)
    check(lib.vbg_avgpool2_fwd(P(x), B, H, W, C_, P(y), _stream()), "vbg_avgpool2_fwd")
    return y


def avgpool2_bwd(dy, H, W):
    B, _, _, C_ = dy.shape
    dx = torch.empty((B, H, W, C_), device=dy.device, dtype=f32)
    check(lib.vbg_avgpool2_bwd(P(dy), B, H, W, C_, P(dx), _stream()), "vbg_avgpool2_bwd")
    return dx


def upsample2_add(lo, skip):
    B, H, W, C_ = skip.shape
    y = torch.empty_like(skip)
    check(lib.vbg_upsample2_add(P(lo), P(skip), B, H, W, C_, P(y), _stream()), "vbg_upsample2_add")
    return y


def sumpool(hi, f, out=None, accumulate=False):
    B, H, W, C_ = hi.shape
    if out is None:
        out = torch.empty((B, H // f, W // f, C_), device=hi.device, dtype=f32)
        accumulate = False
    elif accumulate:
        _untag(out)
    check(lib.vbg_sumpool(P(hi), B, H, W, C_, f, P(out), int(accumulate), _stream()), "vbg_sumpool")
    return out


def nchw_to_nhwc(x):
    B, C_, H, W = x.shape
    y = torch.empty((B, H, W, C_), device=x.device, dtype=f32)
    check(lib.vbg_nchw_to_nhwc(P(x), B, C_, H * W, P(y), _stream()), "vbg_nchw_to_nhwc")
    return y


def nhwc_to_nchw(x):
    B, H, W, C_ = x.shape
    y = torch.empty((B, C_, H, W), device=x.device, dtype=f32)
    check(lib.vbg_nhwc_to_nchw(P(x), B, C_, H * W, P(y), _stream()), "vbg_nhwc_to_nchw")
    return y


def upsample_nhwc_to_nchw(x, f):
    B, h, w, C_ = x.shape
    y = torch.empty((B, C_, h * f, w * f), device=x.device, dtype=f32)
    check(lib.vbg_upsample_nhwc_to_nchw(P(x), B, h, w, C_, f, P(y), _stream()), "vbg_upsample_nhwc_to_nchw")
    return y


def normalize_resize(img, oh, ow, mean, std, batch, b):
    _, h, w = img.shape
    _, H, W, _ = batch.shape
# ... 222 lines not shown
```

Measured before the change: 258.0.

## Store BN-ReLU sign bitmask and use it for backward ReLU masking

BN apply kernels (plain and fold) can now also write a packed 1-bit-per-element ReLU sign mask, built with wave shuffles. The backward reduce and apply kernels read this bitmask instead of the full fp32 output tensor to mask gradients, cutting backward memory traffic and letting the fp32 output be freed earlier. The backward reduce also gets its own rows-per-block heuristic targeting a 256-1024 block grid. This adds an extra small write in the forward pass, requires C divisible by 32, and enables the path by default via an environment flag.

```diff
diff --git a/include/vbg.h b/include/vbg.h
--- a/include/vbg.h
+++ b/include/vbg.h
@@ -256,6 +256,20 @@
 int vbg_bn_bwd_apply_fold(const float* dy, const float* y, const float* x, long long M, int C, const float* mean,
                           const float* invstd, const float* gamma, double* slots, int nslots, double count, int relu, float* dx,
                           float* dres, float* dgamma_accum, float* dbeta_accum, unsigned* dx_amax, void* stream);
+int vbg_bn_apply_sign(const float* x, const float* res, long long M, int C, const float* mean, const float* invstd,
+                      const float* gamma, const float* beta, int relu, float* y, unsigned* sign, unsigned* y_amax, void* stream);
+int vbg_bn_apply_fold_sign(const float* x, const float* res, long long M, int C, double* slots, int nslots, double count,
+                           const double* count_dev, float eps, float momentum, float* mean, float* invstd, float* running_mean,
+                           float* running_var, const float* gamma, const float* beta, int relu, float* y, unsigned* sign,
+                           unsigned* y_amax, void* stream);
+int vbg_bn_bwd_reduce_sign(const float* dy, const unsigned* sign, const float* x, long long M, int C, const float* mean,
+                           const float* invstd, int relu, double* slots_accum, void* stream);
+int vbg_bn_bwd_apply_sign(const float* dy, const unsigned* sign, const float* x, long long M, int C, const float* mean,
+                          const float* invstd, const float* gamma, const double* sums, double count, const double* count_dev,
+                          int relu, float* dx, float* dres, float* dgamma_accum, float* dbeta_accum, unsigned* dx_amax, void* stream);
+int vbg_bn_bwd_apply_fold_sign(const float* dy, const unsigned* sign, const float* x, long long M, int C, const float* mean,
+                               const float* invstd, const float* gamma, double* slots, int nslots, double count, int relu, float* dx,
+                               float* dres, float* dgamma_accum, float* dbeta_accum, unsigned* dx_amax, void* stream);
 int vbg_bn_param_grad(double* slots, int nslots, int clear_slots, int C, double* folded, float* dgamma_accum, float* dbeta_accum,
                       void* stream);
 int vbg_maxpool3x3s2_fwd(const float* x, int B, int H, int W, int C, float* y, int* argmax, void* stream);
@@ -330,6 +344,8 @@
 int vbg_bn_stats_det(const float* x, long long M, int C, double* ws, double* zero_slots, void* stream);
 int vbg_bn_bwd_reduce_det(const float* dy, const float* y, const float* x, long long M, int C, const float* mean,
                           const float* invstd, int relu, double* ws, double* zero_slots, void* stream);
+int vbg_bn_bwd_reduce_det_sign(const float* dy, const unsigned* sign, const float* x, long long M, int C, const float* mean,
+                               const float* invstd, int relu, double* ws, double* zero_slots, void* stream);
 int vbg_embed_ln_bwd_det_blocks(int ntok);
 int vbg_embed_ln_bwd_det(const float* dout, const float* xhat, const float* rstd, int ntok, int hidden, const float* gamma,
                          float drop_p, unsigned long long seed, unsigned long long sid, float* dz_rows, float* part, void* stream);
diff --git a/vibertgrid-pytorch_amd/csrc/convaux.hip b/vibertgrid-pytorch_amd/csrc/convaux.hip
--- a/vibertgrid-pytorch_amd/csrc/convaux.hip
+++ b/vibertgrid-pytorch_amd/csrc/convaux.hip
@@ -11,7 +11,19 @@
 }
 
 constexpr int BN_SLOTS = 32;
-template <bool BWD, bool STORE = false>
+__device__ __forceinline__ void sign_store(const float4& o, long long i, unsigned* __restrict__ sign, bool live = true) {
+    unsigned n = (o.x > 0.f ? 1u : 0u) | (o.y > 0.f ? 2u : 0u) | (o.z > 0.f ? 4u : 0u) | (o.w > 0.f ? 8u : 0u);
+    n <<= ((unsigned)i & 7u) * 4u;
+    n |= __shfl_xor(n, 1, 64);
+    n |= __shfl_xor(n, 2, 64);
+    n |= __shfl_xor(n, 4, 64);
+    if (live && ((unsigned)i & 7u) == 0u) sign[i >> 3] = n;
+}
+__device__ __forceinline__ void sign_mask(float4& g, long long i, const unsigned* __restrict__ sign) {
+    const unsigned n = sign[i >> 3] >> (((unsigned)i & 7u) * 4u);
+    g.x = (n & 1u) ? g.x : 0.f; g.y = (n & 2u) ? g.y : 0.f; g.z = (n & 4u) ? g.z : 0.f; g.w = (n & 8u) ? g.w : 0.f;
+}
+template <bool BWD, bool STORE = false, bool SIGN = false>
 __global__ __launch_bounds__(256) void bn_reduce_kernel(const float* __restrict__ a, const float* __restrict__ y,
                                                         const float* __restrict__ x, long long M, int C,
                                                         const float* __restrict__ mean, const float* __restrict__ invstd,
@@ -37,9 +49,13 @@
                 t.x += v.x * v.x; t.y += v.y * v.y; t.z += v.z * v.z; t.w += v.w * v.w;
             } else {
                 if (relu) {
-                    const float4 yv = reinterpret_cast<const float4*>(y)[o];
-                    v.x = yv.x > 0.f ? v.x : 0.f; v.y = yv.y > 0.f ? v.y : 0.f;
-                    v.z = yv.z > 0.f ? v.z : 0.f; v.w = yv.w > 0.f ? v.w : 0.f;
+                    if (SIGN) {
+                        sign_mask(v, o, reinterpret_cast<const unsigned*>(y));
+                    } else {
+                        const float4 yv = reinterpret_cast<const float4*>(y)[o];
+                        v.x = yv.x > 0.f ? v.x : 0.f; v.y = yv.y > 0.f ? v.y : 0.f;
+                        v.z = yv.z > 0.f ? v.z : 0.f; v.w = yv.w > 0.f ? v.w : 0.f;
+                    }
                 }
                 const float4 xv = reinterpret_cast<const float4*>(x)[o];
                 s.x += v.x; s.y += v.y; s.z += v.z; s.w += v.w;
@@ -73,6 +89,19 @@
 static inline int bn_rows_per_block(long long M, int C) {
     const int C4 = C / 4, QB = C4 < 64 ? C4 : 64, RL = 256 / QB, CG = cdiv(C4, 64);
     long long r = cdiv(M * CG, 512);
+    if (r < 2 * RL) r = 2 * RL;
+    r = cdiv(r, RL) * RL;
+    return (int)r;
+}
+static inline int bn_rows_per_block_bwd(long long M, int C) {
+    const int C4 = C / 4, QB = C4 < 64 ? C4 : 64, RL = 256 / QB, CG = cdiv(C4, 64);
+    long long blocks = M * C * 8 / 65536;
+    if (blocks > 1024) blocks = 1024;
+    if (blocks < 256) blocks = 256;
+#ifdef VBG_BN_BWD_REDUCE_BLOCKS
+    blocks = VBG_BN_BWD_REDUCE_BLOCKS;
+#endif
+    long long r = cdiv(M * CG, blocks);
     if (r < 2 * RL) r = 2 * RL;
     r = cdiv(r, RL) * RL;
     return (int)r;
@@ -124,10 +153,11 @@
     }
 }
 
+template <bool SIGN>
 __global__ void bn_apply_kernel(const float* __restrict__ x, const float* __restrict__ res, long long M, int C4,
                                 const float* __restrict__ mean, const float* __restrict__ invstd,
                                 const float* __restrict__ gamma, const float* __restrict__ beta, int relu,
-                                float* __restrict__ y, unsigned* amax) {
+                                float* __restrict__ y, unsigned* __restrict__ sign, unsigned* amax) {
     const long long total = M * C4;
     const long long stride = (long long)gridDim.x * blockDim.x;
     float mx = 0.f;
@@ -147,11 +177,13 @@
         }
         if (relu) { o.x = fmaxf(o.x, 0.f); o.y = fmaxf(o.y, 0.f); o.z = fmaxf(o.z, 0.f); o.w = fmaxf(o.w, 0.f); }
         reinterpret_cast<float4*>(y)[i] = o;
+        if (SIGN) sign_store(o, i, sign);
         mx = fmaxf(fmaxf(mx, fmaxf(fabsf(o.x), fabsf(o.y))), fmaxf(fabsf(o.z), fabsf(o.w)));
     }
     if (amax) amax_publish(mx, amax);
 }
 
+template <bool SIGN>
 __global__ void bn_bwd_apply_kernel(const float* __restrict__ dy, const float* __restrict__ y, const float* __restrict__ x,
                                     long long M, int C4, int C, const float* __restrict__ mean, const float* __restrict__ invstd,
                                     const float* __restrict__ gamma, const double* __restrict__ sums, double count,
@@ -166,8 +198,12 @@
         const int c4 = (int)(i % C4), c = c4 * 4;
         float4 g = reinterpret_cast<const float4*>(dy)[i];
         if (relu) {
-            const float4 yv = reinterpret_cast<const float4*>(y)[i];
-            g.x = yv.x > 0.f ? g.x : 0.f; g.y = yv.y > 0.f ? g.y : 0.f; g.z = yv.z > 0.f ? g.z : 0.f; g.w = yv.w > 0.f ? g.w : 0.f;
+            if (SIGN) {
+                sign_mask(g, i, reinterpret_cast<const unsigned*>(y));
+            } else {
+                const float4 yv = reinterpret_cast<const float4*>(y)[i];
+                g.x = yv.x > 0.f ? g.x : 0.f; g.y = yv.y > 0.f ? g.y : 0.f; g.z = yv.z > 0.f ? g.z : 0.f; g.w = yv.w > 0.f ? g.w : 0.f;
+            }
         }
         const float4 xv = reinterpret_cast<const float4*>(x)[i];
         const float4 mu = reinterpret_cast<const float4*>(mean)[c4], is = reinterpret_cast<const float4*>(invstd)[c4];
@@ -198,13 +234,15 @@
     }
 }
 
+template <bool SIGN>
 __global__ __launch_bounds__(256) void bn_apply_fold_kernel(const float* __restrict__ x, const float* __restrict__ res, long long M, int C,
                                                             double* __restrict__ slots, int nslots, double count,
                                                             const double* __restrict__ count_dev, float eps, float momentum,
                                                             float* __restrict__ mean_out, float* __restrict__ invstd_out,
                                                             float* __restrict__ running_mean, float* __restrict__ running_var,
                                                             const float* __restrict__ gamma, const float* __restrict__ beta, int relu,
-                                                            int rows_per_block, float* __restrict__ y, unsigned* amax) {
+                                                            int rows_per_block, float* __restrict__ y, unsigned* __restrict__ sign,
+                                                            unsigned* amax) {
     __shared__ double fold[128];
     __shared__ __attribute__((aligned(16))) float cst[4][64];
     const int tid = threadIdx.x, c0 = blockIdx.y * 64;
@@ -234,6 +272,37 @@
     const float4 ga = reinterpret_cast<const float4*>(cst[2])[q], be = reinterpret_cast<const float4*>(cst[3])[q];
     const long long r0 = (long long)blockIdx.x * rows_per_block, r1 = min(M, r0 + rows_per_block);
     float mx = 0.f;
+    if (SIGN) {
+        constexpr int FU = 2;
+        for (long long rb = r0; rb < r1; rb += 16 * FU) {
+            float4 xv[FU], rv[FU];
+#pragma unroll
+            for (int u = 0; u < FU; ++u) {
+                const long long r = rb + rl + 16 * u, i = r * C4 + cq;
+                xv[u] = rv[u] = make_float4(0.f, 0.f, 0.f, 0.f);
+                if (r < r1) {
+                    xv[u] = reinterpret_cast<const float4*>(x)[i];
+                    if (res) rv[u] = reinterpret_cast<const float4*>(res)[i];
+                }
+            }
+#pragma unroll
+            for (int u = 0; u < FU; ++u) {
+                const long long r = rb + rl + 16 * u, i = r * C4 + cq;
+                float4 o;
+                o.x = (xv[u].x - mu.x) * is.x * ga.x + be.x; o.y = (xv[u].y - mu.y) * is.y * ga.y + be.y;
+                o.z = (xv[u].z - mu.z) * is.z * ga.z + be.z; o.w = (xv[u].w - mu.w) * is.w * ga.w + be.w;
+                if (res) { o.x += rv[u].x; o.y += rv[u].y; o.z += rv[u].z; o.w += rv[u].w; }
+                if (relu) { o.x = fmaxf(o.x, 0.f); o.y = fmaxf(o.y, 0.f); o.z = fmaxf(o.z, 0.f); o.w = fmaxf(o.w, 0.f); }
+                if (r < r1) {
+                    reinterpret_cast<float4*>(y)[i] = o;
+                    mx = fmaxf(fmaxf(mx, fmaxf(fabsf(o.x), fabsf(o.y))), fmaxf(fabsf(o.z), fabsf(o.w)));
+                }
+                sign_store(o, i, sign, r < r1);
+            }
+        }
+        if (amax) amax_publish_at(mx, amax, blockIdx.x + blockIdx.y * gridDim.x);
+        return;
+    }
 #pragma unroll 4
     for (long long r = r0 + rl; r < r1; r += 16) {
         const long long i = r * C4 + cq;
@@ -252,6 +321,7 @@
     if (amax) amax_publish_at(mx, amax, blockIdx.x + blockIdx.y * gridDim.x);
 }
 
+template <bool SIGN>
 __global__ __launch_bounds__(256) void bn_bwd_apply_fold_kernel(const float* __restrict__ dy, const float* __restrict__ y,
                                                                 const float* __restrict__ x, long long M, int C,
                                                                 const float* __restrict__ mean, const float* __restrict__ invstd,
@@ -280,14 +350,19 @@
     const float4 ga = reinterpret_cast<const float4*>(cst[2])[q], s0 = reinterpret_cast<const float4*>(cst[3])[q];
     const float4 s1 = reinterpret_cast<const float4*>(cst[4])[q];
     const long long r0 = (long long)blockIdx.x * rows_per_block, r1 = min(M, r0 + rows_per_block);
+    constexpr int BU = SIGN ? 8 : 4;
     float mx = 0.f;
-#pragma unroll 4
+#pragma unroll BU
     for (long long r = r0 + rl; r < r1; r += 16) {
         const long long i = r * C4 + cq;
         float4 g = reinterpret_cast<const float4*>(dy)[i];
         if (relu) {
-            const float4 yv = reinterpret_cast<const float4*>(y)[i];
-            g.x = yv.x > 0.f ? g.x : 0.f; g.y = yv.y > 0.f ? g.y : 0.f; g.z = yv.z > 0.f ? g.z : 0.f; g.w = yv.w > 0.f ? g.w : 0.f;
+            if (SIGN) {
+                sign_mask(g, i, reinterpret_cast<const unsigned*>(y));
+            } else {
+                const float4 yv = reinterpret_cast<const float4*>(y)[i];
+                g.x = yv.x > 0.f ? g.x : 0.f; g.y = yv.y > 0.f ? g.y : 0.f; g.z = yv.z > 0.f ? g.z : 0.f; g.w = yv.w > 0.f ? g.w : 0.f;
+            }
         }
         const float4 xv = reinterpret_cast<const float4*>(x)[i];
         float4 o;
@@ -556,7 +631,6 @@
 
 extern "C" int vbg_bn_stats(const float* x, long long M, int C, double* stats_accum, void* stream) {
     VBG_CHECK_ARG(x && stats_accum && M >= 0 && C > 0 && C % 4 == 0 && ALIGNED16(x));
-    VBG_CHECK_ARG(C / 4 <= 64 ? (256 % (C / 4) == 0) : (C / 4) % 64 == 0);
     if (M == 0) return VBG_OK;
     const int rpb = bn_rows_per_block(M, C);
     VBG_LAUNCH((bn_reduce_kernel<false>), dim3(cdiv(C / 4, 64), cdiv(M, rpb)), dim3(256), 0, S_, x, nullptr, nullptr, M, C, nullptr,
@@ -581,8 +655,23 @@
     VBG_CHECK_ARG(ALIGNED16(x) && ALIGNED16(y) && ALIGNED16(mean) && ALIGNED16(invstd) && ALIGNED16(gamma) && ALIGNED16(beta) &&
                   (!res || ALIGNED16(res)));
     if (M == 0) return VBG_OK;
-    VBG_LAUNCH(bn_apply_kernel, dim3(ew_grid(M * (C / 4), 256)), dim3(256), 0, S_, x, res, M, C / 4, mean, invstd, gamma,
-                       beta, relu, y, y_amax);
+    VBG_LAUNCH(bn_apply_kernel<false>, dim3(ew_grid(M * (C / 4), 256)), dim3(256), 0, S_, x, res, M, C / 4, mean, invstd, gamma,
+                       beta, relu, y, (unsigned*)nullptr, y_amax);
+    VBG_LAUNCH_RET();
+}
+
+extern "C" int vbg_bn_apply_sign(const float* x, const float* res, long long M, int C, const float* mean, const float* invstd,
+                                 const float* gamma, const float* beta, int relu, float* y, unsigned* sign, unsigned* y_amax, void* stream) {
+    VBG_CHECK_ARG(x && mean && invstd && gamma && beta && y && M >= 0 && C > 0 && C % 32 == 0 && (!relu || sign));
+    VBG_CHECK_ARG(ALIGNED16(x) && ALIGNED16(y) && ALIGNED16(mean) && ALIGNED16(invstd) && ALIGNED16(gamma) && ALIGNED16(beta) &&
+                  (!res || ALIGNED16(res)));
+    if (M == 0) return VBG_OK;
+    if (relu)
+        VBG_LAUNCH(bn_apply_kernel<true>, dim3(ew_grid(M * (C / 4), 256)), dim3(256), 0, S_, x, res, M, C / 4, mean, invstd, gamma,
+                   beta, relu, y, sign, y_amax);
+    else
+        VBG_LAUNCH(bn_apply_kernel<false>, dim3(ew_grid(M * (C / 4), 256)), dim3(256), 0, S_, x, res, M, C / 4, mean, invstd, gamma,
+                   beta, relu, y, (unsigned*)nullptr, y_amax);
     VBG_LAUNCH_RET();
 }
 
@@ -590,11 +679,21 @@
                                  const float* invstd, int relu, double* sums_accum, void* stream) {
     VBG_CHECK_ARG(dy && x && mean && invstd && sums_accum && M >= 0 && C > 0 && (!relu || y) && C % 4 == 0);
     VBG_CHECK_ARG(ALIGNED16(dy) && ALIGNED16(x) && ALIGNED16(mean) && ALIGNED16(invstd) && (!relu || ALIGNED16(y)));
-    VBG_CHECK_ARG(C / 4 <= 64 ? (256 % (C / 4) == 0) : (C / 4) % 64 == 0);
     if (M == 0) return VBG_OK;
-    const int rpb = bn_rows_per_block(M, C);
+    const int rpb = bn_rows_per_block_bwd(M, C);
     VBG_LAUNCH((bn_reduce_kernel<true>), dim3(cdiv(C / 4, 64), cdiv(M, rpb)), dim3(256), 0, S_, dy, y, x, M, C, mean, invstd, relu,
                rpb, sums_accum);
+    VBG_LAUNCH_RET();
+}
+
+extern "C" int vbg_bn_bwd_reduce_sign(const float* dy, const unsigned* sign, const float* x, long long M, int C, const float* mean,
+                                      const float* invstd, int relu, double* sums_accum, void* stream) {
+    VBG_CHECK_ARG(dy && x && mean && invstd && sums_accum && M >= 0 && C > 0 && (!relu || sign) && C % 32 == 0);
+    VBG_CHECK_ARG(ALIGNED16(dy) && ALIGNED16(x) && ALIGNED16(mean) && ALIGNED16(invstd));
+    if (M == 0) return VBG_OK;
+    const int rpb = bn_rows_per_block_bwd(M, C);
+    VBG_LAUNCH((bn_reduce_kernel<true, false, true>), dim3(cdiv(C / 4, 64), cdiv(M, rpb)), dim3(256), 0, S_, dy,
+               reinterpret_cast<const float*>(sign), x, M, C, mean, invstd, relu, rpb, sums_accum);
     VBG_LAUNCH_RET();
 }
 
@@ -605,8 +704,22 @@
     VBG_CHECK_ARG(dy && x && mean && invstd && gamma && sums && dx && M >= 0 && C > 0 && (count > 0 || count_dev) && (!relu || y));
     VBG_CHECK_ARG(C % 4 == 0 && ALIGNED16(dy) && ALIGNED16(x) && ALIGNED16(dx) && ALIGNED16(mean) && ALIGNED16(invstd) &&
                   ALIGNED16(gamma) && (!relu || ALIGNED16(y)) && (!dres || ALIGNED16(dres)));
-    if (M > 0) VBG_LAUNCH(bn_bwd_apply_kernel, dim3(ew_grid(M * (C / 4), 256)), dim3(256), 0, S_, dy, y, x, M, C / 4, C, mean, invstd,
+    if (M > 0) VBG_LAUNCH(bn_bwd_apply_kernel<false>, dim3(ew_grid(M * (C / 4), 256)), dim3(256), 0, S_, dy, y, x, M, C / 4, C, mean, invstd,
                           gamma, sums, count, count_dev, relu, dx, dres, dx_amax);
+    if (dgamma_accum && dbeta_accum)
+        VBG_LAUNCH(bn_param_grad_kernel, dim3(cdiv(C, 256)), dim3(256), 0, S_, const_cast<double*>(sums), 1, 0, C, (double*)nullptr, dgamma_accum, dbeta_accum, -1.0);
+    VBG_LAUNCH_RET();
+}
+
+extern "C" int vbg_bn_bwd_apply_sign(const float* dy, const unsigned* sign, const float* x, long long M, int C, const float* mean,
+                                     const float* invstd, const float* gamma, const double* sums, double count,
+                                     const double* count_dev, int relu, float* dx, float* dres, float* dgamma_accum,
+                                     float* dbeta_accum, unsigned* dx_amax, void* stream) {
+    VBG_CHECK_ARG(dy && x && mean && invstd && gamma && sums && dx && M >= 0 && C > 0 && (count > 0 || count_dev) && (!relu || sign));
+    VBG_CHECK_ARG(C % 32 == 0 && ALIGNED16(dy) && ALIGNED16(x) && ALIGNED16(dx) && ALIGNED16(mean) && ALIGNED16(invstd) &&
+                  ALIGNED16(gamma) && (!dres || ALIGNED16(dres)));
+    if (M > 0) VBG_LAUNCH(bn_bwd_apply_kernel<true>, dim3(ew_grid(M * (C / 4), 256)), dim3(256), 0, S_, dy, reinterpret_cast<const float*>(sign), x,
+                          M, C / 4, C, mean, invstd, gamma, sums, count, count_dev, relu, dx, dres, dx_amax);
     if (dgamma_accum && dbeta_accum)
         VBG_LAUNCH(bn_param_grad_kernel, dim3(cdiv(C, 256)), dim3(256), 0, S_, const_cast<double*>(sums), 1, 0, C, (double*)nullptr, dgamma_accum, dbeta_accum, -1.0);
     VBG_LAUNCH_RET();
@@ -624,8 +737,24 @@
     VBG_CHECK_ARG(x && y && slots && mean && invstd && gamma && beta && M > 0 && C > 0 && C % 64 == 0 && nslots >= 1 && (count > 0 || count_dev));
     VBG_CHECK_ARG((running_mean == nullptr) == (running_var == nullptr) && ALIGNED16(x) && ALIGNED16(y) && (!res || ALIGNED16(res)));
     const int rpb = bn_fold_rows(M, C);
-    VBG_LAUNCH(bn_apply_fold_kernel, dim3(cdiv(M, rpb), C / 64), dim3(256), 0, S_, x, res, M, C, slots, nslots, count, count_dev, eps, momentum, mean, invstd,
-               running_mean, running_var, gamma, beta, relu, rpb, y, y_amax);
+    VBG_LAUNCH(bn_apply_fold_kernel<false>, dim3(cdiv(M, rpb), C / 64), dim3(256), 0, S_, x, res, M, C, slots, nslots, count, count_dev, eps, momentum, mean, invstd,
+               running_mean, running_var, gamma, beta, relu, rpb, y, (unsigned*)nullptr, y_amax);
+    VBG_LAUNCH_RET();
+}
+
+extern "C" int vbg_bn_apply_fold_sign(const float* x, const float* res, long long M, int C, double* slots, int nslots, double count,
+                                      const double* count_dev, float eps, float momentum, float* mean, float* invstd, float* running_mean,
+                                      float* running_var, const float* gamma, const float* beta, int relu, float* y, unsigned* sign,
+                                      unsigned* y_amax, void* stream) {
+    VBG_CHECK_ARG(x && y && slots && mean && invstd && gamma && beta && M > 0 && C > 0 && C % 64 == 0 && nslots >= 1 && (count > 0 || count_dev));
+    VBG_CHECK_ARG((running_mean == nullptr) == (running_var == nullptr) && ALIGNED16(x) && ALIGNED16(y) && (!res || ALIGNED16(res)) && (!relu || sign));
+    const int rpb = bn_fold_rows(M, C);
+    if (relu)
+        VBG_LAUNCH(bn_apply_fold_kernel<true>, dim3(cdiv(M, rpb), C / 64), dim3(256), 0, S_, x, res, M, C, slots, nslots, count, count_dev, eps, momentum, mean,
+                   invstd, running_mean, running_var, gamma, beta, relu, rpb, y, sign, y_amax);
+    else
+        VBG_LAUNCH(bn_apply_fold_kernel<false>, dim3(cdiv(M, rpb), C / 64), dim3(256), 0, S_, x, res, M, C, slots, nslots, count, count_dev, eps, momentum, mean,
+                   invstd, running_mean, running_var, gamma, beta, relu, rpb, y, (unsigned*)nullptr, y_amax);
     VBG_LAUNCH_RET();
 }
 
@@ -636,8 +765,20 @@
     VBG_CHECK_ARG(((dgamma_accum == nullptr) == (dbeta_accum == nullptr)) && ALIGNED16(dy) && ALIGNED16(x) && ALIGNED16(dx) &&
                   (!relu || ALIGNED16(y)) && (!dres || ALIGNED16(dres)));
     const int rpb = bn_fold_rows(M, C);
-    VBG_LAUNCH(bn_bwd_apply_fold_kernel, dim3(cdiv(M, rpb), C / 64), dim3(256), 0, S_, dy, y, x, M, C, mean, invstd, gamma, slots, nslots, count,
+    VBG_LAUNCH(bn_bwd_apply_fold_kernel<false>, dim3(cdiv(M, rpb), C / 64), dim3(256), 0, S_, dy, y, x, M, C, mean, invstd, gamma, slots, nslots, count,
                relu, rpb, dx, dres, dgamma_accum, dbeta_accum, dx_amax);
+    VBG_LAUNCH_RET();
+}
+
+extern "C" int vbg_bn_bwd_apply_fold_sign(const float* dy, const unsigned* sign, const float* x, long long M, int C, const float* mean,
+                                          const float* invstd, const float* gamma, double* slots, int nslots, double count, int relu, float* dx,
+                                          float* dres, float* dgamma_accum, float* dbeta_accum, unsigned* dx_amax, void* stream) {
+    VBG_CHECK_ARG(dy && x && mean && invstd && gamma && slots && dx && M > 0 && C > 0 && C % 64 == 0 && nslots >= 1 && count > 0 && (!relu || sign));
+    VBG_CHECK_ARG(((dgamma_accum == nullptr) == (dbeta_accum == nullptr)) && ALIGNED16(dy) && ALIGNED16(x) && ALIGNED16(dx) &&
+                  (!dres || ALIGNED16(dres)));
+    const int rpb = bn_fold_rows(M, C);
+    VBG_LAUNCH(bn_bwd_apply_fold_kernel<true>, dim3(cdiv(M, rpb), C / 64), dim3(256), 0, S_, dy, reinterpret_cast<const float*>(sign), x, M, C, mean, invstd,
+               gamma, slots, nslots, count, relu, rpb, dx, dres, dgamma_accum, dbeta_accum, dx_amax);
     VBG_LAUNCH_RET();
 }
 
@@ -775,12 +916,12 @@
 
 extern "C" int vbg_bn_det_ws_rows(long long M, int C) {
     if (M <= 0 || C <= 0 || C % 4 != 0) return 0;
-    return cdiv(M, bn_rows_per_block(M, C));
+    const int a = cdiv(M, bn_rows_per_block(M, C)), b = cdiv(M, bn_rows_per_block_bwd(M, C));
+    return a > b ? a : b;
 }
 
 extern "C" int vbg_bn_stats_det(const float* x, long long M, int C, double* ws, double* zero_slots, void* stream) {
     VBG_CHECK_ARG(x && ws && zero_slots && M >= 0 && C > 0 && C % 4 == 0 && ALIGNED16(x));
-    VBG_CHECK_ARG(C / 4 <= 64 ? (256 % (C / 4) == 0) : (C / 4) % 64 == 0);
     if (M == 0) return VBG_OK;
     const int rpb = bn_rows_per_block(M, C), nblk = cdiv(M, rpb);
     VBG_LAUNCH((bn_reduce_kernel<false, true>), dim3(cdiv(C / 4, 64), nblk), dim3(256), 0, S_, x, nullptr, nullptr, M, C, nullptr,
@@ -793,11 +934,22 @@
                                      const float* invstd, int relu, double* ws, double* zero_slots, void* stream) {
     VBG_CHECK_ARG(dy && x && mean && invstd && ws && zero_slots && M >= 0 && C > 0 && (!relu || y) && C % 4 == 0);
     VBG_CHECK_ARG(ALIGNED16(dy) && ALIGNED16(x) && ALIGNED16(mean) && ALIGNED16(invstd) && (!relu || ALIGNED16(y)));
-    VBG_CHECK_ARG(C / 4 <= 64 ? (256 % (C / 4) == 0) : (C / 4) % 64 == 0);
     if (M == 0) return VBG_OK;
-    const int rpb = bn_rows_per_block(M, C), nblk = cdiv(M, rpb);
+    const int rpb = bn_rows_per_block_bwd(M, C), nblk = cdiv(M, rpb);
     VBG_LAUNCH((bn_reduce_kernel<true, true>), dim3(cdiv(C / 4, 64), nblk), dim3(256), 0, S_, dy, y, x, M, C, mean, invstd, relu,
                rpb, ws);
     VBG_LAUNCH(bn_det_fold_kernel, dim3(cdiv(2 * C, 256)), dim3(256), 0, S_, ws, nblk, 2 * C, zero_slots);
     VBG_LAUNCH_RET();
 }
+
+extern "C" int vbg_bn_bwd_reduce_det_sign(const float* dy, const unsigned* sign, const float* x, long long M, int C, const float* mean,
+                                          const float* invstd, int relu, double* ws, double* zero_slots, void* stream) {
+    VBG_CHECK_ARG(dy && x && mean && invstd && ws && zero_slots && M >= 0 && C > 0 && (!relu || sign) && C % 32 == 0);
+    VBG_CHECK_ARG(ALIGNED16(dy) && ALIGNED16(x) && ALIGNED16(mean) && ALIGNED16(invstd));
+    if (M == 0) return VBG_OK;
+    const int rpb = bn_rows_per_block_bwd(M, C), nblk = cdiv(M, rpb);
+    VBG_LAUNCH((bn_reduce_kernel<true, true, true>), dim3(cdiv(C / 4, 64), nblk), dim3(256), 0, S_, dy, reinterpret_cast<const float*>(sign), x, M, C,
+               mean, invstd, relu, rpb, ws);
+    VBG_LAUNCH(bn_det_fold_kernel, dim3(cdiv(2 * C, 256)), dim3(256), 0, S_, ws, nblk, 2 * C, zero_slots);
+    VBG_LAUNCH_RET();
+}
diff --git a/vibertgrid-pytorch_amd/csrc/gemm_planes.hip b/vibertgrid-pytorch_amd/csrc/gemm_planes.hip
--- a/vibertgrid-pytorch_amd/csrc/gemm_planes.hip
+++ b/vibertgrid-pytorch_amd/csrc/gemm_planes.hip
@@ -714,11 +714,8 @@
 
 __global__ __launch_bounds__(256) void split_planes_pair_kernel(const float* __restrict__ x, long long ldx, int rows, int cols,
                                                                  unsigned short* __restrict__ out, int ldp, long long plane,
-                                                                 const unsigned* amax, float* colsum) {
-    extern __shared__ float sh_cols[];
+                                                                 const unsigned* amax) {
     const float sc = amax ? vbg_pow2_scale(vbg_amax_read(amax)).x : 1.f;
-    float cs[8] = {0.f, 0.f, 0.f, 0.f, 0.f, 0.f, 0.f, 0.f};
-    const long long i0 = (long long)blockIdx.x * blockDim.x + threadIdx.x;
     const int cpr = ldp / 8;
     const long long n = (long long)rows * cpr;
     const long long stride = (long long)gridDim.x * blockDim.x;
@@ -735,26 +732,66 @@
             for (int t = 0; t < 8; ++t) e[t] = (c + t < cols) ? x[(long long)r * ldx + c + t] : 0.f;
         }
 #pragma unroll
-        for (int t = 0; t < 8; ++t) { cs[t] += e[t]; e[t] *= sc; }
+        for (int t = 0; t < 8; ++t) e[t] *= sc;
         uint4 h, l;
         pg_split2(e[0], e[1], h.x, l.x); pg_split2(e[2], e[3], h.y, l.y); pg_split2(e[4], e[5], h.z, l.z); pg_split2(e[6], e[7], h.w, l.w);
         unsigned short* o = out + (long long)r * ldp + c;
         *reinterpret_cast<uint4*>(o) = h;
         *reinterpret_cast<uint4*>(o + plane) = l;
     }
-    if (colsum) {
-        for (int c = threadIdx.x; c < ldp; c += blockDim.x) sh_cols[c] = 0.f;
-        __syncthreads();
-        if (i0 < n) {
-            const int c = (int)(i0 % cpr) * 8;
-#pragma unroll
-            for (int t = 0; t < 8; ++t) atomicAdd(&sh_cols[c + t], cs[t]);
-        }
-        __syncthreads();
-        for (int c = threadIdx.x; c < cols; c += blockDim.x) {
-            const float v = sh_cols[c];
-            if (v != 0.f) unsafeAtomicAdd(colsum + c, v);
-        }
+}
+
+constexpr int PSC_CH = 32, PSC_RL = 8, PSC_U = 4, PSC_ROWS = PSC_RL * PSC_U;
+__global__ __launch_bounds__(256) void split_planes_pair_colsum_kernel(const float* __restrict__ x, long long ldx, int rows, int cols,
+                                                                        unsigned short* __restrict__ out, int ldp, long long plane,
+                                                                        const unsigned* amax, float* colsum) {
+    __shared__ __attribute__((aligned(16))) float sh_part[PSC_RL][PSC_CH * 8 + 8];
+    const float sc = amax ? vbg_pow2_scale(vbg_amax_read(amax)).x : 1.f;
+    const int cl = threadIdx.x % PSC_CH, rl = threadIdx.x / PSC_CH;
+    const int cpr = ldp / 8, ch = blockIdx.x * PSC_CH + cl, c = ch * 8;
+    const bool live = ch < cpr;
+    const bool vec = ((ldx & 3) == 0) && ((((uintptr_t)x) & 15) == 0) && c + 8 <= cols;
+    const int nrb = (rows + PSC_ROWS - 1) / PSC_ROWS;
+    float cs[8] = {0.f, 0.f, 0.f, 0.f, 0.f, 0.f, 0.f, 0.f};
+    for (int rb = blockIdx.y; rb < nrb; rb += gridDim.y) {
+        const int rbase = rb * PSC_ROWS + rl;
+        float e[PSC_U][8];
+#pragma unroll
+        for (int u = 0; u < PSC_U; ++u) {
+            const int r = rbase + u * PSC_RL;
+            if (live && r < rows && vec) {
+                const float4 a = *reinterpret_cast<const float4*>(x + (long long)r * ldx + c);
+                const float4 b = *reinterpret_cast<const float4*>(x + (long long)r * ldx + c + 4);
+                e[u][0] = a.x; e[u][1] = a.y; e[u][2] = a.z; e[u][3] = a.w; e[u][4] = b.x; e[u][5] = b.y; e[u][6] = b.z; e[u][7] = b.w;
+            } else {
+#pragma unroll
+                for (int t = 0; t < 8; ++t) e[u][t] = (live && r < rows && c + t < cols) ? x[(long long)r * ldx + c + t] : 0.f;
+            }
+        }
+#pragma unroll
+        for (int u = 0; u < PSC_U; ++u) {
+            const int r = rbase + u * PSC_RL;
+#pragma unroll
+            for (int t = 0; t < 8; ++t) { cs[t] += e[u][t]; e[u][t] *= sc; }
+            uint4 h, l;
+            pg_split2(e[u][0], e[u][1], h.x, l.x); pg_split2(e[u][2], e[u][3], h.y, l.y);
+            pg_split2(e[u][4], e[u][5], h.z, l.z); pg_split2(e[u][6], e[u][7], h.w, l.w);
+            if (live && r < rows) {
+                unsigned short* o = out + (long long)r * ldp + c;
+                *reinterpret_cast<uint4*>(o) = h;
+                *reinterpret_cast<uint4*>(o + plane) = l;
+            }
+        }
+    }
+    *reinterpret_cast<float4*>(&sh_part[rl][cl * 8]) = make_float4(cs[0], cs[1], cs[2], cs[3]);
+    *reinterpret_cast<float4*>(&sh_part[rl][cl * 8 + 4]) = make_float4(cs[4], cs[5], cs[6], cs[7]);
+    __syncthreads();
+    const int col = blockIdx.x * (PSC_CH * 8) + threadIdx.x;
+    if (col < cols) {
+        float v = 0.f;
+#pragma unroll
+        for (int k = 0; k < PSC_RL; ++k) v += sh_part[k][threadIdx.x];
+        if (v != 0.f) unsafeAtomicAdd(colsum + col, v);
     }
 }
 
@@ -1056,25 +1093,20 @@
     VBG_CHECK_ARG(rows >= 0 && cols >= 0 && ldp % 32 == 0 && ldp >= cols && plane >= (long long)rows * ldp && plane % 8 == 0);
     if (rows == 0 || cols == 0) return VBG_OK;
     VBG_CHECK_ARG(x && out && ((uintptr_t)out & 15) == 0);
+    if (colsum_accum) {
+        const int panels = cdiv(ldp / 8, PSC_CH), nrb = cdiv(rows, PSC_ROWS);
+        int gy = 2048 / panels;
+        if (gy < 1) gy = 1;
+        if (gy > nrb) gy = nrb;
+        VBG_CHECK_ARG(panels <= 65535);
+        VBG_LAUNCH(split_planes_pair_colsum_kernel, dim3((unsigned)panels, (unsigned)gy), dim3(256), 0, (hipStream_t)stream, x, ldx, rows, cols, out, ldp,
+                   plane, amax, colsum_accum);
+        VBG_LAUNCH_RET();
+    }
     const long long n = (long long)rows * (ldp / 8);
     long long g = (n + 255) / 256;
-    size_t lds = 0;
-    if (colsum_accum) {
-        VBG_CHECK_ARG(ldp * 4 <= 64 * 1024);
-        const long long cpr = ldp / 8;
-        long long a = cpr, b = 256;
-        while (b) { const long long t = a % b; a = b; b = t; }
-        const long long unit = cpr / a;
-        long long k = 288 / unit;
-        if (k < 1) k = 1;
-        const long long need = (g + unit - 1) / unit;
-        if (k > need) k = need;
-        g = k * unit;
-        lds = (size_t)ldp * 4;
-    } else if (g > 256 * 16) {
-        g = 256 * 16;
-    }
-    VBG_LAUNCH(split_planes_pair_kernel, dim3((unsigned)g), dim3(256), lds, (hipStream_t)stream, x, ldx, rows, cols, out, ldp, plane, amax, colsum_accum);
+    if (g > 256 * 16) g = 256 * 16;
+    VBG_LAUNCH(split_planes_pair_kernel, dim3((unsigned)g), dim3(256), 0, (hipStream_t)stream, x, ldx, rows, cols, out, ldp, plane, amax);
     VBG_LAUNCH_RET();
 }
 
diff --git a/vibertgrid-pytorch_amd/vbg/functions.py b/vibertgrid-pytorch_amd/vbg/functions.py
--- a/vibertgrid-pytorch_amd/vbg/functions.py
+++ b/vibertgrid-pytorch_amd/vbg/functions.py
@@ -337,11 +337,13 @@
         M = z2.shape[0]
         r2 = None if res is None else _c(res).view(-1, C)
         y_amax = ops.amax_slot(x.device) if (ops.conv3_f16_enabled() or (any(ctx.needs_input_grad) and ops.conv3_f16_bwd_enabled())) else None
+        sign = ops.bn_sign_empty(M, C, x.device) if (relu and any(ctx.needs_input_grad) and ops.bn_signbits_ok(C)) else None
         if fold:
             if stats is None:
                 stats = ops.bn_stats(z2, ops.bn_zero_slots(x.device, C))
             count, count_dev = float(M), None
-            y, mean, invstd = ops.bn_apply_fold(z2, r2, stats, count, eps, momentum, running_mean, running_var, gamma, beta, relu, y_amax=y_amax)
+            y, mean, invstd = ops.bn_apply_fold(z2, r2, stats, count, eps, momentum, running_mean, running_var, gamma, beta, relu, y_amax=y_amax,
+                                                sign_out=sign)
             y = y.view(z.shape)
         else:
             if training:
@@ -354,7 +356,7 @@
                     count_dev = glob[2 * C:]
                     if ops.bn_fold_ok(C):
                         y, mean, invstd = ops.bn_apply_fold(z2, r2, glob, count, eps, momentum, running_mean, running_var, gamma, beta, relu,
-                                                            y_amax=y_amax, nslots=1, count_dev=count_dev)
+                                                            y_amax=y_amax, nslots=1, count_dev=count_dev, sign_out=sign)
                         y = y.view(z.shape)
                     else:
                         mean, invstd = ops.bn_finalize(glob, C, 1, count, eps, momentum, running_mean, running_var, count_dev)
@@ -363,14 +365,15 @@
             else:
                 mean, invstd, count, count_dev = running_mean, _frozen_invstd(running_var, eps), float(M), None
             if not (training and sync and ops.bn_fold_ok(C)):
-                y = ops.bn_apply(z2, r2, mean, invstd, gamma, beta, relu, y_amax=y_amax).view(z.shape)
+                y = ops.bn_apply(z2, r2, mean, invstd, gamma, beta, relu, y_amax=y_amax, sign_out=sign).view(z.shape)
         if y_amax is not None:
             y._vbg_amax = (y_amax, y._version)
         ctx.fold = fold
         ctx.side_ok = SIDE_OK[0]
         ctx.cfg = (stride, pad, relu, training, count, res is not None, sync)
         ctx.w_ref, ctx.affine = w, (gamma, beta)
-        ctx.save_for_backward(x, w4, col, z, y if relu else None, mean, invstd, gamma, count_dev)
+        ctx.signbits = sign is not None
+        ctx.save_for_backward(x, w4, col, z, sign if sign is not None else (y if relu else None), mean, invstd, gamma, count_dev)
         return y
 
     @staticmethod
@@ -380,25 +383,25 @@
         C = z.shape[-1]
         dy2 = _c(dy).view(-1, C)
         z2 = z.view(-1, C)
-        y2 = None if y is None else y.view(-1, C)
+        sign, y2 = (y, None) if ctx.signbits else (None, None if y is None else y.view(-1, C))
         B_, H_, W_, Cin_ = x.shape
         want_amax = (ctx.needs_input_grad[0] and ops.conv3_f16_bwd_ok(B_, H_, W_, C, Cin_, w4.shape[1], w4.shape[2], stride, pad)) or \
             (col is None and ops.conv3_f16_wgrad_ok(B_, H_, W_, Cin_, C, w4.shape[1], w4.shape[2], stride, pad))
         dz_amax = ops.amax_slot(dy2.device) if want_amax else None
         dgamma, dbeta, sunk = _affine_dest(*ctx.affine)
         if ctx.fold and ops.bn_fold_ok(C, sync):
-            slots = ops.bn_bwd_reduce(dy2, y2, z2, mean, invstd, relu, ops.bn_zero_slots(dy2.device, C))
-            dz2, dres2 = ops.bn_bwd_apply_fold(dy2, y2, z2, mean, invstd, gamma, slots, count, relu, has_res, dgamma, dbeta, dx_amax=dz_amax)
+            slots = ops.bn_bwd_reduce(dy2, y2, z2, mean, invstd, relu, ops.bn_zero_slots(dy2.device, C), sign=sign)
+            dz2, dres2 = ops.bn_bwd_apply_fold(dy2, y2, z2, mean, invstd, gamma, slots, count, relu, has_res, dgamma, dbeta, dx_amax=dz_amax, sign=sign)
             dgamma, dbeta = _affine_done(*ctx.affine, dgamma, dbeta, sunk)
             return ConvBnFn._finish_backward(ctx, dz2, dres2, dz_amax, dgamma, dbeta)
-        slots = ops.bn_bwd_reduce(dy2, y2, z2, mean, invstd, relu)
+        slots = ops.bn_bwd_reduce(dy2, y2, z2, mean, invstd, relu, sign=sign)
         sums = ops.bn_param_grad(slots, C, dgamma, dbeta)
         dgamma, dbeta = _affine_done(*ctx.affine, dgamma, dbeta, sunk)
         if not training:
             sums = torch.zeros_like(sums)
         elif sync:
             SyncCtx.all_reduce(sums)
-        dz2, dres2 = ops.bn_bwd_apply(dy2, y2, z2, mean, invstd, gamma, sums, count, relu, has_res, None, None, count_dev, dx_amax=dz_amax)
+        dz2, dres2 = ops.bn_bwd_apply(dy2, y2, z2, mean, invstd, gamma, sums, count, relu, has_res, None, None, count_dev, dx_amax=dz_amax, sign=sign)
         return ConvBnFn._finish_backward(ctx, dz2, dres2, dz_amax, dgamma, dbeta)
 
     @staticmethod
diff --git a/vibertgrid-pytorch_amd/vbg/lib.py b/vibertgrid-pytorch_amd/vbg/lib.py
--- a/vibertgrid-pytorch_amd/vbg/lib.py
+++ b/vibertgrid-pytorch_amd/vbg/lib.py
@@ -162,6 +162,11 @@
     "vbg_bn_apply_fold": (c_int, [c_vp, c_vp, c_ll, c_int, c_vp, c_int, c_d, c_vp, c_f, c_f, c_vp, c_vp, c_vp, c_vp, c_vp, c_vp, c_int, c_vp, c_vp, c_vp]),
     "vbg_bn_fold_count": (c_int, [c_vp, c_int, c_int, c_int, c_vp, c_d, c_vp]),
     "vbg_bn_bwd_apply_fold": (c_int, [c_vp, c_vp, c_vp, c_ll, c_int, c_vp, c_vp, c_vp, c_vp, c_int, c_d, c_int, c_vp, c_vp, c_vp, c_vp, c_vp, c_vp]),
+    "vbg_bn_apply_sign": (c_int, [c_vp, c_vp, c_ll, c_int, c_vp, c_vp, c_vp, c_vp, c_int, c_vp, c_vp, c_vp, c_vp]),
+    "vbg_bn_apply_fold_sign": (c_int, [c_vp, c_vp, c_ll, c_int, c_vp, c_int, c_d, c_vp, c_f, c_f, c_vp, c_vp, c_vp, c_vp, c_vp, c_vp, c_int, c_vp, c_vp, c_vp, c_vp]),
+    "vbg_bn_bwd_reduce_sign": (c_int, [c_vp, c_vp, c_vp, c_ll, c_int, c_vp, c_vp, c_int, c_vp, c_vp]),
+    "vbg_bn_bwd_apply_sign": (c_int, [c_vp, c_vp, c_vp, c_ll, c_int, c_vp, c_vp, c_vp, c_vp, c_d, c_vp, c_int, c_vp, c_vp, c_vp, c_vp, c_vp, c_vp]),
+    "vbg_bn_bwd_apply_fold_sign": (c_int, [c_vp, c_vp, c_vp, c_ll, c_int, c_vp, c_vp, c_vp, c_vp, c_int, c_d, c_int, c_vp, c_vp, c_vp, c_vp, c_vp, c_vp]),
     "vbg_maxpool3x3s2_fwd": (c_int, [c_vp, c_int, c_int, c_int, c_int, c_vp, c_vp, c_vp]),
     "vbg_maxpool3x3s2_bwd": (c_int, [c_vp, c_vp, c_int, c_int, c_int, c_int, c_int, c_int, c_vp, c_vp]),
     "vbg_avgpool2_fwd": (c_int, [c_vp, c_int, c_int, c_int, c_int, c_vp, c_vp]),
@@ -205,6 +210,7 @@
     "vbg_bn_det_ws_rows": (c_int, [c_ll, c_int]),
     "vbg_bn_stats_det": (c_int, [c_vp, c_ll, c_int, c_vp, c_vp, c_vp]),
     "vbg_bn_bwd_reduce_det": (c_int, [c_vp, c_vp, c_vp, c_ll, c_int, c_vp, c_vp, c_int, c_vp, c_vp, c_vp]),
+    "vbg_bn_bwd_reduce_det_sign": (c_int, [c_vp, c_vp, c_vp, c_ll, c_int, c_vp, c_vp, c_int, c_vp, c_vp, c_vp]),
     "vbg_embed_ln_bwd_det_blocks": (c_int, [c_int]),
     "vbg_embed_ln_bwd_det": (c_int, [c_vp, c_vp, c_vp, c_int, c_int, c_vp, c_f, c_ull, c_ull, c_vp, c_vp, c_vp]),
     "vbg_crf_nll_bwd_det": (c_int, [c_vp, c_vp, c_vp, c_int, c_vp, c_int, c_int, c_int, c_vp, c_vp, c_vp, c_vp, c_vp, c_vp]),
diff --git a/vibertgrid-pytorch_amd/vbg/ops.py b/vibertgrid-pytorch_amd/vbg/ops.py
--- a/vibertgrid-pytorch_amd/vbg/ops.py
+++ b/vibertgrid-pytorch_amd/vbg/ops.py
@@ -1606,29 +1606,58 @@
     return ent[0][o:o + n]
 
 
+_BN_SIGNBITS = [os.environ.get("VBG_BN_SIGNBITS", "1") != "0"]
+
+
+def set_bn_signbits(on: bool):
+    _BN_SIGNBITS[0] = bool(on)
+
+
+def bn_signbits_enabled() -> bool:
+    return _BN_SIGNBITS[0]
+
+
+def bn_signbits_ok(C_) -> bool:
+    return _BN_SIGNBITS[0] and C_ % 32 == 0
+
+
+def bn_sign_empty(M, C_, device):
+    return torch.empty((M * C_ // 32,), device=device, dtype=i32)
+
+
 def bn_fold_count(slots, C_, count):
     out = torch.empty((2 * C_ + 1,), device=slots.device, dtype=torch.float64)
     check(lib.vbg_bn_fold_count(P(slots), bn_slots(), 1, C_, P(out), float(count), _stream()), "vbg_bn_fold_count")
     return out
 
 
-def bn_apply_fold(x2d, res2d, slots, count, eps, momentum, running_mean, running_var, gamma, beta, relu, y_amax=None, nslots=None, count_dev=None):
+def bn_apply_fold(x2d, res2d, slots, count, eps, momentum, running_mean, running_var, gamma, beta, relu, y_amax=None, nslots=None, count_dev=None,
+                  sign_out=None):
     M, C_ = x2d.shape
     out = torch.empty_like(x2d)
     mean = torch.empty((C_,), device=x2d.device, dtype=f32)
     invstd = torch.empty_like(mean)
-    check(lib.vbg_bn_apply_fold(P(x2d), P(res2d), M, C_, P(slots), bn_slots() if nslots is None else int(nslots), float(count), P(count_dev), eps, momentum,
-                                P(mean), P(invstd), P(running_mean), P(running_var), P(gamma), P(beta), int(relu), P(out), P(y_amax), _stream()),
-          "vbg_bn_apply_fold")
+    if sign_out is not None:
+        check(lib.vbg_bn_apply_fold_sign(P(x2d), P(res2d), M, C_, P(slots), bn_slots() if nslots is None else int(nslots), float(count), P(count_dev), eps,
+                                         momentum, P(mean), P(invstd), P(running_mean), P(running_var), P(gamma), P(beta), int(relu), P(out), P(sign_out),
+                                         P(y_amax), _stream()), "vbg_bn_apply_fold_sign")
+    else:
+        check(lib.vbg_bn_apply_fold(P(x2d), P(res2d), M, C_, P(slots), bn_slots() if nslots is None else int(nslots), float(count), P(count_dev), eps, momentum,
+                                    P(mean), P(invstd), P(running_mean), P(running_var), P(gamma), P(beta), int(relu), P(out), P(y_amax), _stream()),
+              "vbg_bn_apply_fold")
     if running_var is not None:
         _BN_EPOCH[0] += 1
     return out, mean, invstd
 
 
-def bn_bwd_apply_fold(dy, y, x, mean, invstd, gamma, slots, count, relu, want_dres, dgamma, dbeta, dx_amax=None):
+def bn_bwd_apply_fold(dy, y, x, mean, invstd, gamma, slots, count, relu, want_dres, dgamma, dbeta, dx_amax=None, sign=None):
     M, C_ = x.shape
     dx = torch.empty_like(x)
     dres = torch.empty_like(x) if want_dres else None
+    if sign is not None:
+        check(lib.vbg_bn_bwd_apply_fold_sign(P(dy), P(sign), P(x), M, C_, P(mean), P(invstd), P(gamma), P(slots), bn_slots(), float(count), int(relu), P(dx),
+                                             P(dres), P(dgamma), P(dbeta), P(dx_amax), _stream()), "vbg_bn_bwd_apply_fold_sign")
+        return dx, dres
     check(lib.vbg_bn_bwd_apply_fold(P(dy), P(y), P(x), M, C_, P(mean), P(invstd), P(gamma), P(slots), bn_slots(), float(count), int(relu), P(dx),
                                     P(dres), P(dgamma), P(dbeta), P(dx_amax), _stream()), "vbg_bn_bwd_apply_fold")
     return dx, dres
@@ -1676,34 +1705,49 @@
     return _BN_EPOCH[0]
 
 
-def bn_apply(x2d, res2d, mean, invstd, gamma, beta, relu, out=None, y_amax=None):
+def bn_apply(x2d, res2d, mean, invstd, gamma, beta, relu, out=None, y_amax=None, sign_out=None):
     M, C_ = x2d.shape
     if out is None:
         out = torch.empty_like(x2d)
     _seen("bn:apply")
+    if sign_out is not None:
+        check(lib.vbg_bn_apply_sign(P(x2d), P(res2d), M, C_, P(mean), P(invstd), P(gamma), P(beta), int(relu), P(out), P(sign_out), P(y_amax), _stream()),
+              "vbg_bn_apply_sign")
+        return out
     check(lib.vbg_bn_apply(P(x2d), P(res2d), M, C_, P(mean), P(invstd), P(gamma), P(beta), int(relu), P(out), P(y_amax), _stream()), "vbg_bn_apply")
     return out
 
 
-def bn_bwd_reduce(dy, y, x, mean, invstd, relu, sums=None):
+def bn_bwd_reduce(dy, y, x, mean, invstd, relu, sums=None, sign=None):
     M, C_ = x.shape
     if sums is None:
         sums = _bn_workspace(x.device, C_)
     if _DET[0]:
         ws = _bn_det_ws(x.device, M, C_)
+        _seen("det:bn_reduce")
+        if sign is not None:
+            check(lib.vbg_bn_bwd_reduce_det_sign(P(dy), P(sign), P(x), M, C_, P(mean), P(invstd), int(relu), P(ws), P(sums), _stream()),
+                  "vbg_bn_bwd_reduce_det_sign")
+            return sums
         check(lib.vbg_bn_bwd_reduce_det(P(dy), P(y), P(x), M, C_, P(mean), P(invstd), int(relu), P(ws), P(sums), _stream()),
               "vbg_bn_bwd_reduce_det")
-        _seen("det:bn_reduce")
         return sums
     _seen("fatomic:bn_reduce")
+    if sign is not None:
+        check(lib.vbg_bn_bwd_reduce_sign(P(dy), P(sign), P(x), M, C_, P(mean), P(invstd), int(relu), P(sums), _stream()), "vbg_bn_bwd_reduce_sign")
+        return sums
     check(lib.vbg_bn_bwd_reduce(P(dy), P(y), P(x), M, C_, P(mean), P(invstd), int(relu), P(sums), _stream()), "vbg_bn_bwd_reduce")
     return sums
 
 
-def bn_bwd_apply(dy, y, x, mean, invstd, gamma, sums, count, relu, want_dres, dgamma, dbeta, count_dev=None, dx_amax=None):
+def bn_bwd_apply(dy, y, x, mean, invstd, gamma, sums, count, relu, want_dres, dgamma, dbeta, count_dev=None, dx_amax=None, sign=None):
     M, C_ = x.shape
     dx = torch.empty_like(x)
     dres = torch.empty_like(x) if want_dres else None
+    if sign is not None:
+        check(lib.vbg_bn_bwd_apply_sign(P(dy), P(sign), P(x), M, C_, P(mean), P(invstd), P(gamma), P(sums), float(count), P(count_dev), int(relu), P(dx),
+                                        P(dres), P(dgamma), P(dbeta), P(dx_amax), _stream()), "vbg_bn_bwd_apply_sign")
+        return dx, dres
     check(lib.vbg_bn_bwd_apply(P(dy), P(y), P(x), M, C_, P(mean), P(invstd), P(gamma), P(sums), float(count), P(count_dev), int(relu), P(dx), P(dres),
                                P(dgamma), P(dbeta), P(dx_amax), _stream()), "vbg_bn_bwd_apply")
     return dx, dres
```

Measured after the change: 261.1 (median of 5 runs). +1.2%, better.
